# EBI-Metagenomics/deciphon-old

Measured on AMD Instinct MI355X. Metric: Gcell-updates/sec, higher is better.
Workload: dtype f32

## Files before the change

### deciphon-old_amd/__init__.py

```python
import ctypes as C
import os
import subprocess

import numpy as np

_HERE = os.path.dirname(os.path.abspath(__file__))
ROOT = os.path.dirname(_HERE)
LIB_PATH = os.path.join(_HERE, "libdcp_hip.so")
CSRC = os.path.join(_HERE, "csrc")

RC_OK, RC_END, RC_EFAIL, RC_EINVAL, RC_EIO, RC_ENOMEM, RC_EPARSE, RC_EAPI, RC_EHTTP = range(9)
RC_NAMES = ["RC_OK", "RC_END", "RC_EFAIL", "RC_EINVAL", "RC_EIO", "RC_ENOMEM", "RC_EPARSE",
            "RC_EAPI", "RC_EHTTP"]
ENTRY_DIST_NULL, ENTRY_DIST_UNIFORM, ENTRY_DIST_OCCUPANCY = 0, 1, 2
NCODES = 1364
NDIST = 129
NXTRANS = 13
CORE_SIZE_MAX = 4096
NUM_THREADS = 64

ABI_SYMBOLS = [
    "dcp_profile_new", "dcp_profile_sample", "dcp_profile_del", "dcp_profile_core_size",
    "dcp_profile_from_parts", "dcp_profile_entry_dist", "dcp_profile_epsilon", "dcp_rnd_seed", "dcp_rnd_next",
    "dcp_dist_unique_id", "dcp_dist_init", "dcp_dist_init_from_file", "dcp_dist_free", "dcp_dist_rank",
# ... 201 lines not shown
        "dcp_gpu_seqs_cut_windows": (I, [P, U, U]),
        "dcp_gpu_seqs_windows": (I, [P, C.POINTER(U), C.POINTER(U)]),
        "dcp_gpu_seqs_window_map": (I, [P, P, P, U]),
        "dcp_gpu_db_keep_dists": (I, [P, I]),
        "dcp_gpu_db_has_dists": (I, [P]),
        "dcp_gpu_decode_paths": (I, [P, P, P, U, P, P, P]),
        "dcp_profile_codon_joint": (I, [P, P, U, U, P, C.POINTER(C.c_double)]),
        "dcp_prod_format_row_codes": (C.c_long, [C.c_char_p, C.c_size_t, C.c_int64, C.c_int64, C.c_char_p, C.c_char_p,
                                                 C.c_double, C.c_double, C.c_char_p, C.c_char_p, P, P, U, P, U, P]),
        "dcp_gpu_path_domains": (I, [P, P, P, U, P, P, I, I, P, U, P, P, P, P]),
        "dcp_gpu_path_domains64": (I, [P, P, P, U, P, P, I, I, P, U, P, P, P, P]),
        "dcp_gpu_path_domains_kernel_ms": (F, [P]),
        "dcp_domains_locate": (I, [P, P, U, P, U, U, P, P, P, P, P, P]),
        "dcp_gpu_domains_locate": (I, [P, P, P, U, P, P, P, P]),
        "dcp_domains_merge": (I, [P, P, P, P, P, P, U, P, C.POINTER(U)]),
        "dcp_domains_regions": (I, [P, P, P, P, P, U, P, U, C.c_uint64, C.c_uint32, P, P, P, P, P, P, P, U, C.POINTER(U)]),
        "dcp_domains_locate_regions": (I, [P, P, U, P, U, P, P, P, P, P, P, P]),
        "dcp_gpu_seqs_cut_regions": (I, [P, P, P, P, P, U]),
        "dcp_gpu_seqs_regions": (U, [P]),
        "dcp_gpu_seqs_region_map": (I, [P, P, P, P, U]),
        "dcp_gpu_scan_pairs": (I, [P, C.POINTER(ScanParams), P, P, U]),
        "dcp_seq_random_thresholds": (I, [P, P]),
        "dcp_seq_random": (None, [C.c_uint64, C.c_uint32, U, P, P]),
        "dcp_gpu_seqs_random": (I, [P, U, U, C.c_uint64, P]),
        "dcp_gumbel_fit": (I, [P, U, C.c_size_t, C.POINTER(C.c_double), C.POINTER(C.c_double)]),
        "dcp_gpu_fit_gumbel": (I, [P, P, P, P]),
        "dcp_gpu_db_calibrate": (I, [P, U, U, C.c_uint64, P, I, I, I, P, P, P]),
        "dcp_gpu_calib_kernel_ms": (F, [P, I]),
        "dcp_gumbel_fit_tail": (I, [P, U, C.c_size_t, U, C.POINTER(C.c_double), C.POINTER(C.c_double),
                                    C.POINTER(C.c_double), C.POINTER(C.c_uint)]),
        "dcp_gpu_fit_gumbel_tail": (I, [P, U, P, P, P, P, P]),
        "dcp_gpu_db_calibrate_tail": (I, [P, U, U, C.c_uint64, P, I, I, I, U, P, P, P, P, P]),
        "dcp_gpu_calib_tail_kernel_ms": (F, [P, I]),
        "dcp_gumbel_sf": (C.c_double, [C.c_double, C.c_double, C.c_double]),
        "dcp_hits_evalues": (I, [P, U, P, P, P, U, C.c_double, P]),
        "dcp_hits_evalues64": (I, [P, U, P, P, P, U, C.c_double, P]),
        "dcp_forward_tables": (I, [U, U, P, P, P, P, P, P, U, C.POINTER(C.c_double), C.POINTER(C.c_double)]),
        "dcp_gpu_forward_pairs": (I, [P, I, I, P, P, U, P, P]),
        "dcp_gpu_forward_kernel_ms": (F, [P]),
        "dcp_posterior_tables": (I, [U, U, P, P, P, P, P, P, U, P, P, P, C.POINTER(C.c_double), C.POINTER(C.c_double)]),
        "dcp_posterior_envelopes": (I, [P, U, C.c_double, U, P, P, U, C.POINTER(U)]),
        "dcp_gpu_posterior_pairs": (I, [P, I, I, P, P, U, P, P, P, P, C.c_uint64, P, P]),
        "dcp_gpu_posterior_kernel_ms": (F, [P]),
        "dcp_mea_tables": (I, [U, U, P, P, P, P, P, P, U, P, U, C.POINTER(U), P, C.POINTER(C.c_double), C.POINTER(C.c_double)]),
        "dcp_mea_path_gain": (I, [U, U, P, P, P, P, P, P, U, P, U, C.POINTER(C.c_double), P]),
        "dcp_gpu_mea_pairs": (I, [P, I, I, P, P, U, P, U, P, P, P, P]),
        "dcp_gpu_mea_kernel_ms": (F, [P]),
        "dcp_gpu_forward_dense": (I, [P, I, I]),
        "dcp_fwd_factor_f32": (C.c_double, [C.c_float]),
        "dcp_forward_scaled_tables": (I, [U, U, P, P, P, P, P, P, U, I, C.POINTER(C.c_double), C.POINTER(C.c_double),
                                          C.POINTER(I)]),
        "dcp_forward_scaled_tables_band": (I, [U, U, P, P, P, P, P, P, U, I, I, C.POINTER(C.c_double), C.POINTER(C.c_double),
                                               C.POINTER(I)]),
        "dcp_gpu_forward_pairs_scaled": (I, [P, I, I, P, P, U, P, P]),
        "dcp_gpu_forward_scaled_redo_pairs": (U, [P]),
        "dcp_gpu_forward_scaled_kernel_ms": (F, [P]),
        "dcp_gpu_forward_dense_scaled": (I, [P, I, I]),
        "dcp_gpu_forward_dense_is_scaled": (I, [P]),
        "dcp_gpu_fetch_forward_scores": (I, [P, P, P]),
        "dcp_gpu_forward_dense_kernel_ms": (F, [P]),
        "dcp_exp_tail_fit": (I, [P, U, C.c_size_t, U, C.POINTER(C.c_double), C.POINTER(C.c_double),
                                 C.POINTER(C.c_double), C.POINTER(C.c_uint)]),
        "dcp_gpu_fit_exp_tail": (I, [P, I, U, P, P, P, P, P]),
        "dcp_gpu_exp_tail_kernel_ms": (F, [P, I]),
        "dcp_gpu_db_calibrate_forward": (I, [P, U, U, C.c_uint64, P, I, I, U, P, P, P, P, P]),
        "dcp_exp_sf": (C.c_double, [C.c_double, C.c_double, C.c_double]),
        "dcp_scores_evalues": (I, [P, P, P, U, P, P, P, U, C.c_double, I, P]),
    }
    if hooks:
        sig["dcp_gpu_test_set_redo_cap"] = (I, [P, U])
        sig["dcp_gpu_test_set_rowsweep_variant"] = (I, [P, I, U])
        sig["dcp_gpu_test_set_ring_stall"] = (I, [P, I])
        sig["dcp_gpu_test_set_seg_col_bytes"] = (I, [P, C.c_ulonglong])
        sig["dcp_gpu_test_set_trace_mode"] = (I, [P, I, C.c_ulonglong])
        sig["dcp_gpu_test_fetch_table_span"] = (I, [P, U, P, C.c_ulonglong, C.POINTER(U), C.POINTER(U), C.POINTER(U)])
        sig["dcp_gpu_test_fetch_seq_words"] = (I, [P, U, P, U, C.POINTER(U)])
        sig["dcp_gpu_test_last_rowsweep_plan"] = (I, [P, P, U, C.POINTER(U)])
        sig["dcp_gpu_test_last_pair_launches"] = (I, [P, P, U, C.POINTER(U)])
        sig["dcp_gpu_test_set_forward_waves"] = (I, [P, U])
        sig["dcp_gpu_test_set_dense_round"] = (I, [P, U])
        sig["dcp_gpu_test_set_forward_scale_band"] = (I, [P, U])
        sig["dcp_gpu_test_set_posterior_budget"] = (I, [P, C.c_ulonglong])
        sig["dcp_gpu_test_set_mea_budget"] = (I, [P, C.c_ulonglong])
    for name, (res, args) in sig.items():
        fn = getattr(lib, name)
        fn.restype = res
        fn.argtypes = args
    return lib


lib = _load()
TESTHOOKS_LIB_PATH = os.path.join(os.path.dirname(LIB_PATH), "libdcp_hip_testhooks.so")


def load_testhooks():
    return _load(TESTHOOKS_LIB_PATH, hooks=True)


def _f32(a):
    return np.ascontiguousarray(a, dtype=np.float32)


def _f64(a):
    return np.ascontiguousarray(a, dtype=np.float64)


class ProteinCfg:

    def __init__(self, entry_dist=ENTRY_DIST_OCCUPANCY, epsilon=0.01):
        if not (0.0 <= epsilon <= 1.0):
            raise DcpError(RC_EINVAL, "epsilon out of [0, 1]")
        self.entry_dist = entry_dist
        self.epsilon = float(np.float32(epsilon))
        self.epsilon64 = float(epsilon)


PROTEIN_CFG_DEFAULT = ProteinCfg(ENTRY_DIST_OCCUPANCY, 0.01)


class ProteinProfile:

    def __init__(self, handle):
        if not handle:
            raise DcpError(RC_EINVAL, "profile construction failed")
        self._h = handle

    def __del__(self):
        h, self._h = getattr(self, "_h", None), None
        if h:
            lib.dcp_profile_del(h)

    @classmethod
    def sample(cls, seed, core_size, cfg=PROTEIN_CFG_DEFAULT, accession="accession", precision=32):
        rc = C.c_int(0)
        if precision == 64:
            h = lib.dcp_profile_sample64(accession.encode(), seed, core_size, cfg.entry_dist,
                                         cfg.epsilon64, C.byref(rc))
        elif precision == 32:
            h = lib.dcp_profile_sample(accession.encode(), seed, core_size, cfg.entry_dist,
                                       cfg.epsilon, C.byref(rc))
        else:
            raise DcpError(RC_EINVAL, "precision is 32 or 64")
        if not h:
            raise DcpError(rc.value, "protein_profile_sample")
        return cls(h)

    @classmethod
    def from_params(cls, null_lprobs, match_lprobs, trans, cfg=PROTEIN_CFG_DEFAULT,
                    accession="accession", consensus=None, precision=32):
        if precision not in (32, 64):
            raise DcpError(RC_EINVAL, "precision is 32 or 64")
        cv = _f64 if precision == 64 else _f32
        nl, ml, tr = cv(null_lprobs), cv(match_lprobs), cv(trans)
        M = ml.shape[0] if ml.ndim == 2 else 0
        if nl.shape != (20,) or ml.shape != (M, 20) or tr.shape != (M + 1, 7):
            raise DcpError(RC_EINVAL, "bad parameter shapes")
        rc = C.c_int(0)
        cons = consensus.encode() if consensus else None
        new, eps = (lib.dcp_profile_new64, cfg.epsilon64) if precision == 64 else (lib.dcp_profile_new, cfg.epsilon)
        h = new(accession.encode(), M, cfg.entry_dist, eps, nl.ctypes.data, ml.ctypes.data, tr.ctypes.data, cons,
                C.byref(rc))
        if not h:
            raise DcpError(rc.value, "protein_model_setup")
        return cls(h)

    @property
# ... 922 lines not shown
                                                           lam.ctypes.data, status.ctypes.data, tau.ctypes.data,
                                                           k_eff.ctypes.data))
        self._seq_lens = np.full(n, length, np.int64)
        return mu, lam, status, tau, k_eff

    def test_set_dense_round(self, npairs):
        self._check(self._lib.dcp_gpu_test_set_dense_round(self._c, int(npairs)))

    def posterior_pairs(self, seq_idx, profile_idx, multi_hits=True, hmmer3_compat=False):
        sq, pr = _pair_list(seq_idx, profile_idx)
        lens = getattr(self, "_seq_lens", np.zeros(0, np.int64))
        ok = sq < len(lens)
        cap = int(np.sum(lens[sq[ok]] + 1)) if len(sq) else 0
        row_off = np.zeros(len(sq) + 1, np.uint64)
        begin, end, core = (np.zeros(cap, np.float64) for _ in range(3))
        fwd, bwd = np.zeros(len(sq), np.float64), np.zeros(len(sq), np.float64)
        self._check(self._lib.dcp_gpu_posterior_pairs(self._c, int(multi_hits), int(hmmer3_compat), sq.ctypes.data,
                                                      pr.ctypes.data, len(sq), row_off.ctypes.data, begin.ctypes.data,
                                                      end.ctypes.data, core.ctypes.data, cap, fwd.ctypes.data,
                                                      bwd.ctypes.data))
        return row_off, begin, end, core, fwd, bwd

    @property
    def posterior_kernel_ms(self):
        return self._lib.dcp_gpu_posterior_kernel_ms(self._c)

    def test_set_posterior_budget(self, nbytes):
        self._check(self._lib.dcp_gpu_test_set_posterior_budget(self._c, int(nbytes)))

    def mea_pairs(self, seq_idx, profile_idx, multi_hits=True, hmmer3_compat=False):
        sq, pr = _pair_list(seq_idx, profile_idx)
        n = len(sq)
        lens = self._seq_lens
        sizes = np.array([p.core_size for p in self._profiles or []], np.int64)
        ok = (sq < len(lens)) & (pr < len(sizes))
        cap = int(np.sum(lens[sq[ok]] + sizes[pr[ok]] + 16))
        off = np.zeros(n + 1, np.uint32)
        gain, fwd = np.zeros(n, np.float64), np.zeros(n, np.float64)
        for _ in range(2):
            steps, post = np.zeros(max(cap, 1), STEP_DTYPE), np.zeros(max(cap, 1), np.float64)
            rc = self._lib.dcp_gpu_mea_pairs(self._c, int(multi_hits), int(hmmer3_compat), sq.ctypes.data, pr.ctypes.data, n,
                                             steps.ctypes.data, cap, off.ctypes.data, post.ctypes.data, gain.ctypes.data,
                                             fwd.ctypes.data)
            if rc != RC_ENOMEM or int(off[n]) <= cap:
                break
            cap = int(off[n])
        self._check(rc)
        paths = [steps[int(off[i]):int(off[i + 1])].copy() for i in range(n)]
        posts = [post[int(off[i]):int(off[i + 1])].copy() for i in range(n)]
        return paths, posts, gain, fwd

    @property
    def mea_kernel_ms(self):
        return self._lib.dcp_gpu_mea_kernel_ms(self._c)

    def test_set_mea_budget(self, nbytes):
        self._check(self._lib.dcp_gpu_test_set_mea_budget(self._c, int(nbytes)))

    def set_hit_buffer(self, hits_dev_ptr, cap, nhits_dev_ptr):
        self._check(self._lib.dcp_gpu_set_hit_buffer(self._c, hits_dev_ptr, cap, nhits_dev_ptr))

    def set_hit_buffer64(self, hits_dev_ptr, cap, nhits_dev_ptr):
        self._check(self._lib.dcp_gpu_set_hit_buffer64(self._c, hits_dev_ptr, cap, nhits_dev_ptr))

    def hit_buffer64(self):
        h, n, cap = C.c_void_p(), C.c_void_p(), C.c_uint(0)
        self._check(self._lib.dcp_gpu_hit_buffer64(self._c, C.byref(h), C.byref(n), C.byref(cap)))
        return h.value, n.value, cap.value

    def launch_infos(self):
        out = []
        for i in range(self.last_scan_launches):
            li = LaunchInfo()
            self._check(self._lib.dcp_gpu_last_scan_launch_info(self._c, i, C.byref(li)))
            out.append(dict(R=li.nodes_per_lane, W=li.waves_per_pair, nprofiles=li.nprofiles,
                            ms=li.ms, cells=li.cells, algorithmic_bytes=li.algorithmic_bytes))
        return out

    def sync(self):
        self._check(self._lib.dcp_gpu_sync(self._c))

    def test_set_redo_cap(self, cap):
        self._check(self._lib.dcp_gpu_test_set_redo_cap(self._c, int(cap)))

    def test_set_ring_stall(self, on):
        self._check(self._lib.dcp_gpu_test_set_ring_stall(self._c, int(bool(on))))

    def test_set_seg_col_bytes(self, nbytes):
        self._check(self._lib.dcp_gpu_test_set_seg_col_bytes(self._c, int(nbytes)))

    def test_set_trace_mode(self, own_forward, budget_floats=0):
        self._check(self._lib.dcp_gpu_test_set_trace_mode(self._c, int(bool(own_forward)), int(budget_floats)))

    def test_table_span(self, p):
        span, ldk, eb = C.c_uint(0), C.c_uint(0), C.c_uint(0)
        self._check(self._lib.dcp_gpu_test_fetch_table_span(self._c, p, None, 0, C.byref(span), C.byref(ldk),
                                                            C.byref(eb)))
        out = np.zeros((NCODES, span.value), np.float64 if eb.value == 8 else np.float32)
        self._check(self._lib.dcp_gpu_test_fetch_table_span(self._c, p, out.ctypes.data, out.nbytes, C.byref(span),
                                                            C.byref(ldk), C.byref(eb)))
        return out, ldk.value

    def test_rowsweep_plan(self):
        n = C.c_uint(0)
        rc = self._lib.dcp_gpu_test_last_rowsweep_plan(self._c, None, 0, C.byref(n))
        if rc != RC_ENOMEM:
            self._check(rc or RC_EFAIL)
        w = np.zeros(n.value, np.uint32)
        self._check(self._lib.dcp_gpu_test_last_rowsweep_plan(self._c, w.ctypes.data, len(w), C.byref(n)))
        per = (len(w) - 2) // int(w[1])
        classes = {}
        for k in range(int(w[1])):
            R, W, path, stage, waves, pf, chunk, redo, rest = (int(v) for v in w[2 + per * k:2 + per * k + 9])
            if path:
                classes[(R, W)] = dict(path=("plain", "mp", "segmented")[path - 1], stage=stage, waves=waves, prefetch=pf,
                                       chunk=chunk, seg_redo=redo, flagged_rest=bool(rest))
        return dict(forked=bool(w[0]), classes=classes)

    def test_pair_launches(self):
        n = C.c_uint(0)
        rc = self._lib.dcp_gpu_test_last_pair_launches(self._c, None, 0, C.byref(n))
        if rc != RC_ENOMEM:
            self._check(rc or RC_EFAIL)
        w = np.zeros(n.value, np.uint32)
        self._check(self._lib.dcp_gpu_test_last_pair_launches(self._c, w.ctypes.data, len(w), C.byref(n)))
        out = []
        for i in range(int(w[0])):
            kind, prec, a, b, units, tpb, cap = (int(v) for v in w[1 + 7 * i:8 + 7 * i])
            rec = dict(kind=("scan_pairs", "qlane_redo", "seg_redo")[kind - 1], precision=prec, units=units, tpb=tpb, cap=cap)
            rec.update(dict(cls=(a, b)) if prec == 32 else dict(group=a, R=b))
            out.append(rec)
        return out

    def test_set_rowsweep_variant(self, stage_rows, block_waves=0):
        self._check(self._lib.dcp_gpu_test_set_rowsweep_variant(self._c, int(stage_rows), int(block_waves)))

    @property
    def last_scan_ms(self):
        return self._lib.dcp_gpu_last_scan_ms(self._c)

    @property
    def last_scan_kernel(self):
        return self._lib.dcp_gpu_last_scan_kernel(self._c)

    @property
    def last_scan_launches(self):
        return self._lib.dcp_gpu_last_scan_launches(self._c)

    @property
    def last_scan_query_plan(self):
        nb, rows, prow, mg = C.c_uint(0), C.c_ulonglong(0), C.c_uint(0), C.c_uint(0)
        self._check(self._lib.dcp_gpu_last_scan_query_plan(self._c, C.byref(nb), C.byref(rows), C.byref(prow),
                                                           C.byref(mg)))
        return dict(nblocks=nb.value, sum_block_rows=rows.value, plane_rows=prow.value,
                    max_groups_per_slot=mg.value)

    @property
    def last_scan_redo_pairs(self):
        n = C.c_uint(0)
        self._check(self._lib.dcp_gpu_last_scan_redo_pairs(self._c, C.byref(n)))
        return n.value

    @property
    def cells(self):
        return self._lib.dcp_gpu_scan_cells(self._c)

# ... 110 lines not shown
```

### deciphon-old_amd/csrc/dcp_gpu.hip

```cpp
#include "dcp_kernels.h"
#include "dcp_f64.h"
#include "dcp_seqs.h"
#include "dcp_decode.h"
#include "dcp_domains.h"
#include "dcp_calib.h"
#include "dcp_forward.h"
#include "dcp_forward_scaled.h"
#include "dcp_mea.h"
#include "dcp_posterior.h"
#include "dcp_test_hooks.h"

#include <hip/hip_runtime.h>

#include <algorithm>
#include <cmath>
#include <cstdarg>
#include <cstdio>
#include <cstring>
#include <limits>
#include <map>
#include <new>
#include <numeric>
#include <string>
#include <queue>
// ... 48 lines not shown
    }
    hipError_t reserve(size_t count) { return n < count ? alloc(count) : hipSuccess; }
    void release()
    {
        if (p) (void)hipFree(p);
        p = nullptr;
        n = 0;
    }
    ~DevBuf() { release(); }
};

template <class Real, class Hit> struct ScanResults
{
    DevBuf<Real> d_null, d_alt;
    DevBuf<Hit> d_hits;
    DevBuf<unsigned> d_nhits;
    unsigned hit_cap = 0;
    bool have_scores = false;
    Hit *ext_hits = nullptr;
    unsigned *ext_nhits = nullptr;
    unsigned ext_cap = 0;
    Hit *hits() const { return ext_hits ? ext_hits : d_hits.p; }
    unsigned *nhits() const { return ext_hits ? ext_nhits : d_nhits.p; }
    unsigned cap() const { return ext_hits ? ext_cap : hit_cap; }
    hipError_t ensure(size_t npairs, bool keep_scores)
    {
        hipError_t e = hipSuccess;
        if (keep_scores && d_null.n != npairs)
        {
            if ((e = d_null.alloc(npairs)) != hipSuccess) return e;
            if ((e = d_alt.alloc(npairs)) != hipSuccess) return e;
        }
        have_scores = keep_scores;
        unsigned const want_cap = (unsigned)std::min<size_t>(npairs, (size_t)1 << 22);
        if (!ext_hits && hit_cap < want_cap)
        {
            if ((e = d_hits.alloc(want_cap)) != hipSuccess) return e;
            hit_cap = want_cap;
        }
        return d_nhits.p ? hipSuccess : d_nhits.alloc(1);
    }
    void release()
    {
        d_null.release(), d_alt.release(), d_hits.release(), d_nhits.release();
        hit_cap = 0;
        have_scores = false;
    }
};

bool is_nan(float v)
{
    uint32_t bits;
    std::memcpy(&bits, &v, sizeof bits);
    return (bits & 0x7fffffffu) > 0x7f800000u;
}
bool is_nan(double v)
{
    uint64_t bits;
    std::memcpy(&bits, &v, sizeof bits);
    return (bits & 0x7fffffffffffffffull) > 0x7ff0000000000000ull;
}

constexpr int kMaxLaunches = 2 * kNumClasses + 1;

struct LastScan
{
    bool scanned = false;
    bool f64 = false;
    bool pair_scan = false;
    unsigned q0 = 0, q1 = 0;
    int kernel = 0;
    int kernel_variant = 0;
    struct dcp_scan_params prm = {};
    unsigned launches = 0;
    unsigned n_launched = 0;
    int launched_class[kMaxLaunches] = {0};
    bool launched_redo[kMaxLaunches] = {false};
    bool overlapped = false;
    unsigned redo_pairs = 0;
    uint64_t pair_cells = 0, pair_bytes = 0;
    uint64_t pair_class_cells[DCP_MAX_CLASSES] = {0}, pair_class_bytes[DCP_MAX_CLASSES] = {0};
    bool redo_pending = false, redo_pending64 = false, ring_check_pending = false;
#ifdef DCP_TEST_HOOKS
    struct RowsweepClassPlan
    {
        unsigned path = 0;
        unsigned stage = 0, waves = 0, prefetch = 0;
        unsigned chunk = 0;
        unsigned flagged_rest = 0;
    } rs_plan[kNumClasses];
    struct PairLaunch
    {
        unsigned kind, precision, a, b, units, tpb, cap;
    };
    std::vector<PairLaunch> pair_launches;
#endif
};

}

struct dcp_gpu_ctx
{
    int device = 0;
    hipStream_t stream = nullptr;
    hipEvent_t ev_start = nullptr, ev_stop = nullptr;
    std::string err;

    unsigned nprof = 0;
    std::vector<dcp_prof_meta> metas;
    std::vector<unsigned> core_sizes;
    unsigned class_first[kNumClasses + 1] = {0};
    DevBuf<dcp_prof_meta> d_metas;
    DevBuf<uint32_t> d_slot_of_pidx;
    std::vector<uint32_t> slot_of_pidx;
    DevBuf<float> d_emis_match, d_emis_insert, d_emis_null, d_trans8;
    DevBuf<float> d_dists, d_eps;
    std::vector<dcp_expand_tile> rs_tiles;
    uint64_t rs_floats = 0;
    bool rs_ready = false;
    bool one_layout = false;
    uint64_t table_bytes = 0;
    int ql_G = 2;
    std::vector<dcp_ql_prof> ql_metas;
    uint64_t sum_core = 0, sum_tiles = 0;
    uint64_t class_core[DCP_MAX_CLASSES] = {0};
    unsigned max_tiles = 0;
    DevBuf<dcp_ql_prof> d_ql_metas;
    DevBuf<float> d_emis_tiles, d_ttrans, d_scratch;
    DevBuf<uint32_t> d_qorder;
    DevBuf<uint32_t> d_words_t, d_wt_off;
    std::vector<dcp_mp_group> mp_groups;
    unsigned mp_first[3] = {0, 0, 0};
    unsigned mp_flagged_first[2] = {0, 0};
    DevBuf<dcp_mp_group> d_mp_groups;
    DevBuf<float> d_mp_in;
    bool mp_in_ready = false;
    DevBuf<dcp_ql_group> d_ql_groups;
    DevBuf<uint32_t> d_slot_first;
    unsigned ql_nqb = 0, ql_plane_rows = 0;
    unsigned ring_stall = 0;
    uint32_t *h_qstage = nullptr;
    size_t h_qstage_n = 0;
    hipEvent_t ev_qstage = nullptr;
    int rs_force_stg = -1;
    unsigned rs_force_bw = 0;
    unsigned rs_pad_lds = 0;
    int rs_force_pf = 0;
    int rs_force_R = 0;
    bool any_exact_e = false;
    DevBuf<unsigned> d_task_counter;
    DevBuf<dcp_pair> d_redo;
    DevBuf<unsigned> d_redo_n;
    unsigned qorder_q0 = ~0u, qorder_q1 = ~0u, qorder_lmax = 0;
    unsigned num_cus = 0;
    unsigned qorder_nt = 0;
    unsigned redo_cap_limit = 1u << 26;
    float last_ql_ms = 0;

    unsigned nseqs = 0;
    unsigned strands = 0;
    uint64_t total_len = 0;
    std::vector<uint32_t> seq_len;
    unsigned win_window = 0, win_step = 0;
    std::vector<uint32_t> win_src, win_off;
    std::vector<uint32_t> reg_src, reg_begin;
    std::vector<uint8_t> reg_minus;
    void drop_windows()
    {
        win_window = win_step = 0;
        win_src.clear(), win_off.clear();
        reg_src.clear(), reg_begin.clear(), reg_minus.clear();
    }
    DevBuf<uint32_t> d_seq_words, d_seq_woff, d_seq_len;
    DevBuf<float> d_xtrans;
    int xt_multi = -1, xt_h3 = -1;
    bool xt_explicit = false;
    std::vector<double> xt64;

    ScanResults<float, dcp_hit> res;
    LastScan last;
    DevBuf<dcp_pair> d_pair_list;
    DevBuf<unsigned> d_pair_n;
    hipEvent_t ev_class[kMaxLaunches] = {nullptr};
    hipStream_t class_stream[kNumClasses] = {nullptr};
    hipEvent_t ev_trace[kNumClasses + 1] = {nullptr};
    DevBuf<float> d_trace_work;
    int trace_mode = 0;
    uint64_t trace_budget = 0;
    DevBuf<float> d_seg_scratch;
    DevBuf<dcp_pair> d_seg_redo;
    DevBuf<unsigned> d_seg_redo_n;
    int seg_mode = -1;
    int mp_mode = -1;
    uint64_t seg_col_bytes = (uint64_t)6 << 30;

    int precision = 0;
    double lrt_threshold64 = std::numeric_limits<double>::quiet_NaN();
    struct F64Db
    {
        std::vector<dcp_f64_prof> profs;
        std::vector<uint32_t> slot_of_pidx;
        unsigned group_first[5] = {0, 0, 0, 0, 0};
        DevBuf<dcp_f64_prof> d_profs;
        DevBuf<double> d_tab, d_trans, d_xe;
        DevBuf<double> d_xt, d_col;
        ScanResults<double, dcp_hit64> res;
        DevBuf<uint32_t> d_order, d_qorder, d_slot_first;
        DevBuf<dcp_ql_group> d_groups;
        unsigned plan_blocks = 0, plan_rows = 0, plan_max_groups = 0;
        uint64_t plan_sum_rows = 0;
        DevBuf<double> d_planes;
        DevBuf<unsigned> d_task, d_redo_n;
        DevBuf<dcp_f64_pair> d_redo;
        DevBuf<dcp_f64_pair> d_pair_list;
        DevBuf<unsigned> d_pair_n;
        void release()
        {
            d_pair_list.release(), d_pair_n.release();
            profs.clear();
            d_profs.release(), d_tab.release(), d_trans.release(), d_xe.release();
            d_xt.release(), d_col.release(), res.release();
            d_order.release(), d_qorder.release(), d_planes.release(), d_task.release(), d_redo_n.release();
            d_redo.release(), d_slot_first.release(), d_groups.release();
            slot_of_pidx.clear();
        }
    } f64;

    bool keep_dists = false;
    struct DecodeDb
    {
        bool ready = false;
        DevBuf<double> d_dists64;
        DevBuf<uint32_t> d_match_row;
        DevBuf<double> d_exp, d_eps;
        void release()
// ... 2277 lines not shown
    HIP_TRY(c, hipMemcpyAsync(c->d_qorder.p, h_ord, nq * sizeof(uint32_t), hipMemcpyHostToDevice, c->stream));
    HIP_TRY(c, hipMemcpyAsync(c->d_wt_off.p, wt_off, (nqb + 1u) * sizeof(uint32_t), hipMemcpyHostToDevice, c->stream));
    HIP_TRY(c, hipMemcpyAsync(c->d_slot_first.p, h_slots, nslot_words * sizeof(uint32_t), hipMemcpyHostToDevice, c->stream));
    HIP_TRY(c, hipMemcpyAsync(c->d_ql_groups.p, h_groups, ngroup_words * sizeof(uint32_t), hipMemcpyHostToDevice, c->stream));
    HIP_TRY(c, hipEventRecord(c->ev_qstage, c->stream));
    dcp_qlane_args ta{};
    ta.seq_words = a.seq_words, ta.seq_woff = a.seq_woff, ta.seq_len = a.seq_len;
    ta.qorder = c->d_qorder.p, ta.words_t = c->d_words_t.p, ta.wt_off = c->d_wt_off.p;
    ta.groups = c->d_ql_groups.p, ta.slot_first = c->d_slot_first.p;
    ta.nseqs = nq, ta.nqblocks = nqb;
    if (dcp_launch_qlane_transpose(&ta, NTq, c->stream)) return c->fail(DCP_EFAIL, "no kernel for %u-query blocks", NTq);
    HIP_TRY(c, hipGetLastError());
    c->qorder_q0 = q_begin, c->qorder_q1 = q_end, c->qorder_nt = NTq;
    c->ql_nqb = nqb, c->ql_plane_rows = plan.plane_rows + 8u;
    return DCP_OK;
}

static int record_launch(dcp_gpu_ctx *c, int k, bool is_redo, hipStream_t stream, bool join)
{
    HIP_TRY(c, hipEventRecord(c->ev_class[c->last.n_launched], stream));
    if (join) HIP_TRY(c, hipStreamWaitEvent(c->stream, c->ev_class[c->last.n_launched], 0));
    c->last.launched_redo[c->last.n_launched] = is_redo;
    c->last.launched_class[c->last.n_launched++] = k;
    c->last.launches++;
    return DCP_OK;
}

static int launch_qlane_scan(dcp_gpu_ctx *c, struct dcp_scan_params const *prm, dcp_scan_args &a, unsigned NT,
                             unsigned ql_blocks_per_cu, bool two_stage, bool use_w3)
{
    dcp_qlane_args qa{};
    qa.profs = c->d_ql_metas.p;
    qa.emis_tiles = c->one_layout ? c->d_emis_match.p : c->d_emis_tiles.p;
    qa.tiles_from_rows = c->one_layout ? 1u : 0u;
    qa.emis_insert = c->d_emis_insert.p;
    qa.emis_null = c->d_emis_null.p;
    qa.ttrans = c->d_ttrans.p;
    qa.seq_words = a.seq_words;
    qa.seq_woff = a.seq_woff;
    qa.seq_len = a.seq_len;
    qa.xtrans = a.xtrans;
    qa.qorder = c->d_qorder.p;
    qa.words_t = c->d_words_t.p;
    qa.wt_off = c->d_wt_off.p;
    qa.groups = c->d_ql_groups.p;
    qa.slot_first = c->d_slot_first.p;
    qa.ring_stall = c->ring_stall;
    qa.task_counter = c->d_task_counter.p;
    qa.out_null = a.out_null;
    qa.out_alt = a.out_alt;
    qa.hits = a.hits;
    qa.nhits = a.nhits;
    qa.hit_cap = a.hit_cap;
    qa.lrt_threshold = prm->lrt_threshold;
    qa.nprof = c->nprof;
    qa.nprof_total = c->nprof;
    qa.nseqs = a.nseqs;
    qa.q_base = a.q_base;
    qa.plane_rows = c->ql_plane_rows;
    qa.nqblocks = c->ql_nqb;
    uint64_t const ntasks = (uint64_t)c->nprof * qa.nqblocks;
    if (ntasks > 0xffffffffull) return c->fail(DCP_EINVAL, "scan too large for one launch");
    qa.ntasks = (unsigned)ntasks;
    bool const redo = prm->multi_hits != 0 || c->xt_explicit || (dcp_qlane_exact_e_by_redo() && c->any_exact_e);
    unsigned redo_grid[kNumClasses] = {0};
    if (redo)
    {
        if (int rc = ensure_rowsweep_layout(c)) return rc;
        a.emis_match = c->d_emis_match.p;
        uint64_t tot = 0;
        uint64_t const cap_limit = c->redo_cap_limit;
        for (int k = 0; k < kNumClasses; ++k)
        {
            uint64_t const pairs = (uint64_t)a.nseqs * (c->class_first[k + 1] - c->class_first[k]);
            unsigned const cap = (unsigned)std::min<uint64_t>(pairs, cap_limit);
            qa.redo_base[k] = (unsigned)tot;
            qa.redo_cap[k] = cap;
            tot += cap;
            uint64_t const tpb = dcp_rowsweep_tasks_per_block(kClasses[k].W);
            uint64_t g = std::min<uint64_t>((cap + tpb - 1) / tpb, 8ull * c->num_cus);
            redo_grid[k] = (unsigned)((g + 7) / 8 * 8);
        }
        HIP_TRY(c, c->d_redo.reserve((size_t)tot));
    }
    HIP_TRY(c, c->d_redo_n.reserve(DCP_MAX_CLASSES + 2));
    HIP_TRY(c, hipMemsetAsync(c->d_redo_n.p, 0, (DCP_MAX_CLASSES + 2) * sizeof(unsigned), c->stream));
    qa.redo = c->d_redo.p;
    qa.redo_n = c->d_redo_n.p;
    qa.redo_overflow = c->d_redo_n.p + DCP_MAX_CLASSES;
    qa.ring_error = c->d_redo_n.p + DCP_MAX_CLASSES + 1;
    uint64_t const per_block = (uint64_t)dcp_qlane_scratch_planes() * (uint64_t)qa.plane_rows * NT;
    uint64_t const budget = (uint64_t)64 << 28;
    uint64_t fit = per_block ? budget / per_block : 0;
    uint64_t const resident_blocks = (uint64_t)ql_blocks_per_cu * c->num_cus;
    unsigned nblocks = (unsigned)std::min<uint64_t>(std::min<uint64_t>(ntasks, resident_blocks), fit);
    if (use_w3) nblocks = (nblocks + 2u) / 3u * 3u;
    if (nblocks == 0)
        return c->fail(DCP_ENOMEM, "sequences too long for the query-lane kernel (%u plane rows): use kernel = 1", qa.plane_rows);
    size_t const need = (size_t)nblocks * per_block;
    HIP_TRY(c, c->d_scratch.reserve(need));
    qa.scratch = c->d_scratch.p;
    HIP_TRY(c, hipMemsetAsync(c->d_task_counter.p, 0, sizeof(unsigned), c->stream));
    HIP_TRY(c, hipEventRecord(c->ev_start, c->stream));
    if (two_stage ? dcp_launch_qlane2(&qa, nblocks, c->stream)
                  : use_w3 ? dcp_launch_qlane_w3(&qa, nblocks / 3u, c->stream)
                           : dcp_launch_qlane(&qa, nblocks, NT, c->stream))
        return c->fail(DCP_EFAIL, "query-lane launch failed");
    HIP_TRY(c, hipGetLastError());
    if (int rc = record_launch(c, -1, false, c->stream, false)) return rc;
    for (int k = 0; redo && k < kNumClasses; ++k)
    {
        if (redo_grid[k] == 0) continue;
        a.pairs = c->d_redo.p + qa.redo_base[k];
        a.npairs = c->d_redo_n.p + k;
        a.pair_cap = qa.redo_cap[k];
        a.first_prof = 0;
        a.nprof = c->nprof;
        SizeClass const sc = kClasses[k];
        if (dcp_launch_rowsweep(sc.R, sc.W, &a, redo_grid[k], c->stream))
            return c->fail(DCP_EFAIL, "no kernel for class R=%d W=%d", sc.R, sc.W);
        if (int rc = record_launch(c, k, true, c->stream, false)) return rc;
        note_pair_launch(c, DCP_PL_QLANE_REDO, 32u, (unsigned)sc.R, (unsigned)sc.W, redo_grid[k], dcp_rowsweep_tasks_per_block(sc.W), a.pair_cap);
    }
    HIP_TRY(c, hipGetLastError());
    HIP_TRY(c, hipEventRecord(c->ev_stop, c->stream));
    c->last.redo_pending = redo;
    c->last.ring_check_pending = two_stage;
    c->last.scanned = true;
    return DCP_OK;
}

struct SegSweepPlan
{
    unsigned stride = 0;
    unsigned chunk[kNumClasses] = {0};
    uint64_t redo_off[kNumClasses] = {0}, col_rows = 0, redo_tot = 0;
};
static SegSweepPlan plan_segsweep(dcp_gpu_ctx const *c, unsigned q_begin, unsigned q_end)
{
    SegSweepPlan sp;
    unsigned const nq = q_end - q_begin;
    sp.stride = *std::max_element(c->seq_len.begin() + q_begin, c->seq_len.begin() + q_end) + 2u;
    for (int k = 0; k < kNumClasses; ++k)
    {
        unsigned const np = c->class_first[k + 1] - c->class_first[k];
        SizeClass const sc = kClasses[k];
        uint64_t const pairs = (uint64_t)np * nq;
        bool const want = c->seg_mode == 1 || (c->seg_mode < 0 && pairs >= 16ull * c->num_cus);
        bool const have = sc.W > 1 && want && np > 0 && pairs <= ((uint64_t)1 << 26);
        if (!have) continue;
        uint64_t const per_query = (uint64_t)np * 2u * sp.stride * 16u;
        uint64_t const chunk = std::min<uint64_t>(nq, c->seg_col_bytes / per_query);
        if (chunk == 0) continue;
        if ((uint64_t)np * ((chunk + 3u) / 4u) > 0x7ffffff0ull) continue;
        sp.chunk[k] = (unsigned)chunk;
        sp.col_rows += (uint64_t)np * chunk * 2u * sp.stride;
        sp.redo_off[k] = sp.redo_tot, sp.redo_tot += pairs;
    }
    return sp;
}

static int launch_segsweep_class(dcp_gpu_ctx *c, dcp_scan_args &a, int k, SegSweepPlan const &sp, float *col_base,
                                 hipStream_t ls, bool overlap)
{
    unsigned const first = a.first_prof, last = first + a.nprof, np = a.nprof, chunk = sp.chunk[k], nq = a.nseqs;
    uint64_t const ntasks = (uint64_t)a.nprof * a.nchunks;
    SizeClass const sc = kClasses[k];
    a.seg_stride = sp.stride;
    a.seg_redo = c->d_seg_redo.p + sp.redo_off[k];
    a.seg_redo_n = c->d_seg_redo_n.p + k;
    a.seg_redo_cap = (unsigned)ntasks;
    for (unsigned sub = first; sub < last;)
    {
        unsigned const segR = seg_r_of(c->metas[sub].core_size);
        unsigned sub_end = sub, max_m = 0;
        while (sub_end < last && seg_r_of(c->metas[sub_end].core_size) == segR)
            max_m = std::max(max_m, c->metas[sub_end].core_size), ++sub_end;
        unsigned const nsub = sub_end - sub, nseg_max = (max_m + 64u * segR - 1u) / (64u * segR);
        a.first_prof = sub, a.nprof = nsub;
        a.seg_col0 = col_base + (size_t)(sub - first) * chunk * 2u * sp.stride * 4u;
        a.seg_col1 = a.seg_col0 + (size_t)nsub * chunk * sp.stride * 4u;
        for (unsigned qc = 0; qc < nq; qc += chunk)
        {
            a.seg_q0 = qc, a.seg_nq = std::min(chunk, nq - qc);
            for (unsigned sg = 0; sg < nseg_max; ++sg)
            {
                a.seg_index = sg;
                if (dcp_launch_segsweep((int)segR, &a, dcp_segsweep_blocks(nsub, a.seg_nq), ls))
                    return c->fail(DCP_EFAIL, "no segmented kernel for %u nodes per lane", segR);
            }
        }
        sub = sub_end;
    }
    a.first_prof = first, a.nprof = np;
    if (int rc = record_launch(c, k, false, ls, false)) return rc;
    a.pairs = a.seg_redo, a.npairs = a.seg_redo_n, a.pair_cap = a.seg_redo_cap;
    a.first_prof = 0, a.nprof = c->nprof;
    uint64_t g = std::min<uint64_t>(ntasks, 8ull * c->num_cus);
    g = (g + 7u) / 8u * 8u;
    if (dcp_launch_rowsweep(sc.R, sc.W, &a, (unsigned)g, ls))
        return c->fail(DCP_EFAIL, "no kernel for class R=%d W=%d", sc.R, sc.W);
    note_pair_launch(c, DCP_PL_SEG_REDO, 32u, (unsigned)sc.R, (unsigned)sc.W, (unsigned)g, dcp_rowsweep_tasks_per_block(sc.W), a.pair_cap);
    return record_launch(c, k, true, ls, overlap);
}

static int launch_rowsweep_scan(dcp_gpu_ctx *c, dcp_scan_args &a, unsigned q_begin, unsigned q_end)
{
    unsigned const nq = q_end - q_begin;
// ... 979 lines not shown
    if (segmented) HIP_TRY(c, hipMemcpy(redo, c->d_seg_redo_n.p, sizeof redo, hipMemcpyDeviceToHost));
    out[0] = c->last.overlapped ? 1u : 0u;
    out[1] = (unsigned)kNumClasses;
    for (int k = 0; k < kNumClasses; ++k)
    {
        unsigned *w = out + 2u + DCP_RS_PLAN_WORDS * (unsigned)k;
        LastScan::RowsweepClassPlan const &r = c->last.rs_plan[k];
        w[0] = (unsigned)kClasses[k].R, w[1] = (unsigned)kClasses[k].W, w[2] = r.path, w[3] = r.stage, w[4] = r.waves;
        w[5] = r.prefetch, w[6] = r.chunk, w[7] = r.path == DCP_RS_PATH_SEGMENTED ? redo[k] : 0u, w[8] = r.flagged_rest;
    }
    return DCP_OK;
}
int dcp_gpu_test_last_pair_launches(dcp_gpu_ctx *c, unsigned *out, unsigned cap, unsigned *nwords)
{
    if (!c || !nwords) return DCP_EINVAL;
    if (!c->last.scanned) return c->fail(DCP_EINVAL, "no scan yet");
    *nwords = 1u + DCP_PL_WORDS * (unsigned)c->last.pair_launches.size();
    if (!out || cap < *nwords) return DCP_ENOMEM;
    HIP_TRY(c, hipSetDevice(c->device));
    HIP_TRY(c, hipStreamSynchronize(c->stream));
    out[0] = (unsigned)c->last.pair_launches.size();
    unsigned *w = out + 1u;
    for (LastScan::PairLaunch const &l : c->last.pair_launches)
    {
        w[0] = l.kind, w[1] = l.precision, w[2] = l.a, w[3] = l.b, w[4] = l.units, w[5] = l.tpb, w[6] = l.cap;
        w += DCP_PL_WORDS;
    }
    return DCP_OK;
}
int dcp_gpu_test_set_seg_col_bytes(dcp_gpu_ctx *c, unsigned long long bytes)
{
    if (!c) return DCP_EINVAL;
    c->seg_col_bytes = bytes ? bytes : (uint64_t)6 << 30;
    return DCP_OK;
}
int dcp_gpu_test_set_ring_stall(dcp_gpu_ctx *c, int on)
{
    if (!c) return DCP_EINVAL;
    c->ring_stall = on ? 1u : 0u;
    return DCP_OK;
}
int dcp_gpu_test_set_trace_mode(dcp_gpu_ctx *c, int own_forward, unsigned long long budget_floats)
{
    if (!c) return DCP_EINVAL;
    c->trace_mode = own_forward ? 1 : 0;
    c->trace_budget = budget_floats;
    return DCP_OK;
}
int dcp_gpu_test_set_posterior_budget(dcp_gpu_ctx *c, unsigned long long bytes)
{
    if (!c) return DCP_EINVAL;
    c->sweeps.post_budget = bytes;
    return DCP_OK;
}

int dcp_gpu_test_set_mea_budget(dcp_gpu_ctx *c, unsigned long long bytes)
{
    if (!c) return DCP_EINVAL;
    c->sweeps.mea_budget = bytes;
    return DCP_OK;
}

int dcp_gpu_test_set_forward_waves(dcp_gpu_ctx *c, unsigned nwaves)
{
    if (!c) return DCP_EINVAL;
    c->sweeps.waves_cap = nwaves;
    return DCP_OK;
}

int dcp_gpu_test_set_forward_scale_band(dcp_gpu_ctx *c, unsigned bits)
{
    if (!c || bits > 500u) return DCP_EINVAL;
    c->sweeps.band = (int)bits;
    return DCP_OK;
}

int dcp_gpu_test_set_dense_round(dcp_gpu_ctx *c, unsigned npairs)
{
    if (!c) return DCP_EINVAL;
    c->sweeps.dense_round = npairs;
    return DCP_OK;
}

int dcp_gpu_test_set_redo_cap(dcp_gpu_ctx *c, unsigned cap)
{
    if (!c) return DCP_EINVAL;
    c->redo_cap_limit = cap ? cap : 1u << 26;
    return DCP_OK;
}
int dcp_gpu_test_fetch_table_span(dcp_gpu_ctx *c, unsigned p, void *out, unsigned long long cap_bytes,
                                  unsigned *span, unsigned *ldk, unsigned *elem_bytes)
{
    if (!c || !span || !ldk || !elem_bytes || p >= c->nprof) return DCP_EINVAL;
    HIP_TRY(c, hipSetDevice(c->device));
    void const *src = nullptr;
    unsigned w = 0, ld = 0, eb = 0;
    if (c->precision == 64)
    {
        for (dcp_f64_prof const &m : c->f64.profs)
            if (m.pidx == p) src = c->f64.d_tab.p + m.tab_off, w = m.ldk, ld = m.ldk, eb = sizeof(double);
    }
    else
    {
        if (int rc = ensure_rowsweep_layout(c)) return rc;
        for (dcp_prof_meta const &m : c->metas)
            if (m.pidx == p) src = c->d_emis_match.p + m.emis_off, w = m.width, ld = m.ldk, eb = sizeof(float);
    }
    if (!src) return DCP_EINVAL;
    *span = w, *ldk = ld, *elem_bytes = eb;
    if (!out) return DCP_OK;
    if (cap_bytes < (unsigned long long)DCP_NCODES * w * eb) return c->fail(DCP_ENOMEM, "span needs more room");
    HIP_TRY(c, hipMemcpy2D(out, (size_t)w * eb, src, (size_t)ld * eb, (size_t)w * eb, DCP_NCODES, hipMemcpyDeviceToHost));
    return DCP_OK;
}
#endif

int dcp_gpu_sync(dcp_gpu_ctx *c)
{
    if (!c) return DCP_EINVAL;
    HIP_TRY(c, hipSetDevice(c->device));
    return finish_scan(c);
}

int dcp_gpu_last_scan_redo_pairs(dcp_gpu_ctx *c, unsigned *npairs)
{
    if (!c || !npairs) return DCP_EINVAL;
    if (!c->last.scanned) return c->fail(DCP_EINVAL, "no scan yet");
    HIP_TRY(c, hipSetDevice(c->device));
    if (int rc = finish_scan(c)) return rc;
    *npairs = c->last.redo_pairs;
    return DCP_OK;
}

int dcp_gpu_last_scan_query_plan(dcp_gpu_ctx *c, unsigned *nblocks, unsigned long long *sum_block_rows,
                                 unsigned *plane_rows, unsigned *max_groups_per_slot)
{
    if (!c) return DCP_EINVAL;
    if (!c->last.scanned) return c->fail(DCP_EINVAL, "no scan yet");
    HIP_TRY(c, hipSetDevice(c->device));
    if (int rc = finish_scan(c)) return rc;
    if (!c->last.f64 || c->last.kernel_variant != 4)
        return c->fail(DCP_EINVAL, "the last scan did not run the f64 query-lane kernel (kernel = 4): it has no batch plan");
    if (nblocks) *nblocks = c->f64.plan_blocks;
    if (sum_block_rows) *sum_block_rows = c->f64.plan_sum_rows;
    if (plane_rows) *plane_rows = c->f64.plan_rows;
    if (max_groups_per_slot) *max_groups_per_slot = c->f64.plan_max_groups;
    return DCP_OK;
}

float dcp_gpu_last_scan_ms(dcp_gpu_ctx *c)
{
    if (!c || !c->last.scanned) return -1.0f;
    float ms = -1.0f;
    if (hipEventSynchronize(c->ev_stop) != hipSuccess) return -1.0f;
    if (hipEventElapsedTime(&ms, c->ev_start, c->ev_stop) != hipSuccess) return -1.0f;
    return ms;
}

unsigned dcp_gpu_last_scan_launches(dcp_gpu_ctx const *c) { return c ? c->last.launches : 0; }
int dcp_gpu_last_scan_kernel(dcp_gpu_ctx const *c) { return c && c->last.scanned ? c->last.kernel_variant : 0; }

int dcp_gpu_last_scan_launch_info(dcp_gpu_ctx *c, unsigned i, struct dcp_launch_info *out)
{
    if (!c || !out || !c->last.scanned) return DCP_EINVAL;
    if (i >= c->last.n_launched) return DCP_EINVAL;
    int const k = c->last.launched_class[i];
// ... 742 lines not shown
```

### deciphon-old_amd/csrc/dcp_kernels.h

```cpp
#ifndef DCP_KERNELS_H
#define DCP_KERNELS_H

#include "dcp_host.h"
#include <stdint.h>

struct dcp_prof_meta
{
    uint64_t emis_off;
    uint32_t trans_off;
    uint32_t core_size;
    uint32_t ldk;
    uint32_t pidx;
    uint32_t flags;
    uint32_t width;
};
#define DCP_PROF_EXACT_E 1u

struct dcp_mp_group
{
    uint64_t emis_off;
    uint32_t trans_off;
    uint32_t ldk;
    uint32_t in_off;
    uint32_t nparts;
    uint32_t col0[4];
    uint32_t core_size[4];
    uint32_t pidx[4];
    uint32_t slot[4];
};

struct dcp_pair
{
    uint32_t q;
    uint32_t slot;
};
#define DCP_MAX_CLASSES 16

struct dcp_scan_args
{
    dcp_prof_meta const *profs;
    float const *emis_match;
    float const *emis_insert;
    float const *emis_null;
    float const *trans8;
    uint32_t const *seq_words;
    uint32_t const *seq_woff;
    uint32_t const *seq_len;
    float const *xtrans;
    float *out_null;
    float *out_alt;
    dcp_hit *hits;
    unsigned *nhits;
    unsigned hit_cap;
    float lrt_threshold;
    unsigned first_prof;
    unsigned nprof;
    unsigned nprof_total;
    unsigned nseqs;
    unsigned q_base;
    unsigned qchunk;
    unsigned nchunks;
    dcp_pair const *pairs;
    unsigned const *npairs;
    unsigned pair_cap;
    float *seg_col0, *seg_col1;
    unsigned seg_stride;
    unsigned seg_index;
    dcp_mp_group const *mp_groups;
    float const *mp_in;
    unsigned seg_q0, seg_nq;
    dcp_pair *seg_redo;
    unsigned *seg_redo_n;
    unsigned seg_redo_cap;
    float *trace_work;
    uint64_t const *trace_woff;
    float *trace_alt;
};

struct dcp_expand_tile
{
    uint64_t out_off;
    uint32_t dist_row;
    uint32_t ncols;
    uint32_t nstore;
    uint32_t ld_code;
    uint32_t ld_col;
    uint32_t kt;
    uint32_t col0;
};

enum : uint32_t
{
    DCP_TRACE_NO_PATH = 0xffffffffu,
    DCP_TRACE_TOO_LONG = 0xfffffffeu,
};
struct dcp_trace_args
{
    dcp_prof_meta const *profs;
    uint32_t const *slot_of_pidx;
    float const *emis_match;
    float const *emis_insert;
    float const *emis_null;
    float const *trans8;
    uint32_t const *seq_words;
    uint32_t const *seq_woff;
    uint32_t const *seq_len;
    float const *xtrans;
    dcp_hit const *hits;
    unsigned nhits;
    float *work;
    uint64_t const *work_off;
    dcp_step *steps;
    uint32_t const *step_off;
    uint32_t *nsteps;
    float *alt_out;
    int null_model;
    int skip_forward;
    uint32_t const *work_ld;
};

struct dcp_ql_prof
{
    uint64_t tile_off;
    uint32_t ttrans_off;
    uint32_t core_size;
    uint32_t ntiles;
    uint32_t pidx;
    uint32_t rs_slot;
    uint32_t cls;
    uint32_t needs_exact_e;
    uint32_t ldk;
};

struct dcp_ql_group
{
    uint32_t qfirst;
    uint32_t nq;
    uint32_t rowbase;
    uint32_t lmax;
};

struct dcp_qlane_args
{
    dcp_ql_prof const *profs;
    float const *emis_tiles;
    float const *emis_insert;
    float const *emis_null;
    float const *ttrans;
    uint32_t const *seq_words;
    uint32_t const *seq_woff;
    uint32_t const *seq_len;
    float const *xtrans;
    uint32_t const *qorder;
    dcp_ql_group const *groups;
    uint32_t const *slot_first;
    uint32_t *words_t;
    uint32_t const *wt_off;
    float *scratch;
    unsigned *task_counter;
    unsigned *ring_error;
    unsigned ring_stall;
    dcp_pair *redo;
    unsigned *redo_n;
    unsigned *redo_overflow;
    unsigned redo_base[DCP_MAX_CLASSES];
    unsigned redo_cap[DCP_MAX_CLASSES];
    float *out_null;
    float *out_alt;
    dcp_hit *hits;
    unsigned *nhits;
    unsigned hit_cap;
    float lrt_threshold;
    unsigned nprof;
    unsigned nprof_total;
    unsigned nseqs;
    unsigned q_base;
    unsigned plane_rows;
    unsigned ntasks;
    unsigned nqblocks;
    unsigned tiles_from_rows;
};

struct dcp_expand_args
{
    dcp_expand_tile const *tiles;
    float const *dists;
    float const *eps;
    float *out;
};

#ifdef __cplusplus
extern "C" {
#endif
void dcp_launch_expand(dcp_expand_args const *a, unsigned ntiles, void *stream);
int dcp_launch_rowsweep(int R, int W, dcp_scan_args const *a, unsigned nblocks,
                        void *stream);
unsigned dcp_rowsweep_tasks_per_block(int W);
int dcp_launch_segsweep(int R, dcp_scan_args const *a, unsigned nblocks, void *stream);
int dcp_launch_mp(int K, dcp_scan_args const *a, void *stream);
void dcp_launch_mp_in(dcp_mp_group const *groups, unsigned ngroups, unsigned n_first, unsigned k_first, unsigned k_rest,
                      float const *emis_insert, float const *emis_null, float *out, void *stream);
unsigned dcp_segsweep_blocks(unsigned nprof, unsigned nq);
int dcp_launch_rowsweep_grid(int R, int W, dcp_scan_args const *a, int stg, unsigned bw, void *stream,
                             unsigned pad_lds,
                             int prefetch2);
unsigned dcp_rowsweep_max_block_waves(int R, int W, int stg);
unsigned dcp_rowsweep_stage_bytes(int R, int stg);
int dcp_launch_qlane(dcp_qlane_args const *a, unsigned nblocks, unsigned nt, void *stream);
int dcp_launch_qlane2(dcp_qlane_args const *a, unsigned nblocks, void *stream);
unsigned dcp_qlane2_lds_bytes(void);
int dcp_launch_qlane_w3(dcp_qlane_args const *a, unsigned nblocks, void *stream);
int dcp_launch_qlane_transpose(dcp_qlane_args const *a, unsigned nt, void *stream);
void dcp_launch_trace(dcp_trace_args const *a, unsigned nhits, void *stream);
int dcp_launch_trace_forward(int R, int W, dcp_scan_args const *a, unsigned nblocks, void *stream);
unsigned dcp_qlane_block_size(void);
unsigned dcp_qlane_tile_nodes(void);
unsigned dcp_qlane_scratch_planes(void);
unsigned dcp_qlane_diag_build(void);
unsigned dcp_qlane_group_rows(unsigned lmax);
unsigned dcp_qlane_window_planes(void);
unsigned dcp_qlane_exact_e_by_redo(void);
#ifdef __cplusplus
}
#endif

#ifdef __HIP__
__device__ inline __attribute__((always_inline)) bool dcp_lrt_hit(float nul, float alt, float thr)
{
    auto finite = [](float v) { return (__builtin_bit_cast(unsigned, v) & 0x7f800000u) != 0x7f800000u; };
    float const lrt = -2 * (nul - alt);
    return finite(nul) && finite(alt) && finite(lrt) && !(lrt < thr);
}
#endif

#endif
```

### deciphon-old_amd/csrc/dcp_kernels.hip

```cpp
#include "dcp_kernels.h"

#include <hip/hip_runtime.h>
#include <algorithm>

namespace
{

__device__ __forceinline__ float neg_inf() { return -__builtin_inff(); }

typedef float const __attribute__((address_space(4))) cfloat;
typedef uint32_t const __attribute__((address_space(4))) cu32;
__device__ __forceinline__ cfloat *as_const(float const *p) { return (cfloat *)(unsigned long long)p; }
__device__ __forceinline__ cu32 *as_const(uint32_t const *p) { return (cu32 *)(unsigned long long)p; }

template <int CTRL, int ROW_MASK, int BANK_MASK>
__device__ __forceinline__ float dpp_mov(float old_value, float v)
{
    return __builtin_bit_cast(
        float, __builtin_amdgcn_update_dpp(__builtin_bit_cast(int, old_value),
                                           __builtin_bit_cast(int, v), CTRL,
                                           ROW_MASK, BANK_MASK, false));
}

__device__ __forceinline__ float lane_shr1(float v, float first)
// ... 138 lines not shown
};
template <> struct VecLoad<6>
{
    static __device__ __forceinline__ void ld(float const *p, float (&o)[6])
    {
        float t[3], u[3];
        VecLoad<3>::ld(p, t);
        VecLoad<3>::ld(p + 3, u);
        o[0] = t[0], o[1] = t[1], o[2] = t[2], o[3] = u[0], o[4] = u[1], o[5] = u[2];
    }
};
template <> struct VecLoad<7>
{
    static __device__ __forceinline__ void ld(float const *p, float (&o)[7])
    {
        struct __attribute__((packed, aligned(4))) f4 { float x, y, z, w; };
        f4 v = *reinterpret_cast<f4 const *>(p);
        float u[3];
        VecLoad<3>::ld(p + 4, u);
        o[0] = v.x, o[1] = v.y, o[2] = v.z, o[3] = v.w, o[4] = u[0], o[5] = u[1], o[6] = u[2];
    }
};
template <> struct VecLoad<8>
{
    static __device__ __forceinline__ void ld(float const *p, float (&o)[8])
    {
        float4 v = *reinterpret_cast<float4 const *>(p);
        float4 w = *reinterpret_cast<float4 const *>(p + 4);
        o[0] = v.x, o[1] = v.y, o[2] = v.z, o[3] = v.w, o[4] = w.x, o[5] = w.y, o[6] = w.z, o[7] = w.w;
    }
};

__device__ __forceinline__ unsigned code_of(unsigned w, int l)
{
    constexpr unsigned off[5] = {0u, 4u, 20u, 84u, 340u};
    return off[l - 1] + (w & ((1u << (2 * l)) - 1u));
}

template <int R> struct PairState
{
    float P[5][R];
    float Q[5][R];
    float PX[5];
};

struct LaneSpecial
{
    float a;
    float b;
    float c;
};

template <int R> struct Trans
{
    float ent[R], mm[R], im[R], dm[R], md[R], dd[R], mi[R], ii[R];
};

struct RowOut
{
    float E;
    float X;
};

template <int W> struct Exchange
{
    float m[2][W], i[2][W], d[2][W], e[2][W];
    int flag[3];
};

template <int R, int r = 1>
__device__ __forceinline__ void chain_rest(float const (&a)[R], float (&d)[R], float const (&dd)[R])
{
    if constexpr (r < R)
    {
        d[r] = fmaxf(a[r], d[r - 1] + dd[r]);
        chain_rest<R, r + 1>(a, d, dd);
    }
}

struct NoSink
{
    template <class... A> __device__ __forceinline__ void operator()(A const &...) const {}
};
template <int R, int W, int PH, int PARTS = 1, class Fetch, class Sink = NoSink>
__device__ __forceinline__ RowOut dp_row(PairState<R> &s, Trans<R> const &t,
                                         float (&em)[5][R], float (&em3)[R], float (&em4)[R], float (&em5)[R], float (&eN)[5], float (&eI)[5],
                                         LaneSpecial const &sp, float const xEB,
                                         Exchange<(W > 1 ? W : 1)> *xc,
                                         unsigned wave, unsigned lane,
                                         unsigned &gen, unsigned const exact_e, Fetch &&fetch, Sink &&sink = Sink{})
{
    constexpr int s1 = (PH + 4) % 5, s2 = (PH + 3) % 5, s3 = (PH + 2) % 5,
                  s4 = (PH + 1) % 5, s5 = PH;
    float const ni = neg_inf();

    float m[R], ins[R];
#pragma unroll
    for (int r = 0; r < R; ++r)
    {
        m[r] = max5(s.P[s1][r] + em[0][r], s.P[s2][r] + em[1][r],
                    s.P[s3][r] + em3[r], s.P[s4][r] + em4[r],
                    s.P[s5][r] + em5[r]);
        ins[r] = max5(s.Q[s1][r] + eI[0], s.Q[s2][r] + eI[1], s.Q[s3][r] + eI[2],
                      s.Q[s4][r] + eI[3], s.Q[s5][r] + eI[4]);
    }
    float const X = max5(s.PX[s1] + eN[0], s.PX[s2] + eN[1], s.PX[s3] + eN[2],
                         s.PX[s4] + eN[3], s.PX[s5] + eN[4]);
    __builtin_amdgcn_sched_barrier(0);
    fetch();
    __builtin_amdgcn_sched_barrier(0);

    float E = ni;
    if constexpr (W == 1)
    {
        float em = m[0];
#pragma unroll
        for (int r = 1; r < R; ++r)
            em = fmaxf(em, m[r]);
        if constexpr (PARTS == 1) E = wave_max(em);
        else E = part_max<PARTS>(em);
    }

    float m_first = ni, i_first = ni, d_first = ni;
    constexpr bool XW = W > 1;
    float a[R], d[R];
#pragma unroll
    for (int r = 1; r < R; ++r)
        a[r] = m[r - 1] + t.md[r];
    auto refine = [&]() {
        if constexpr (W == 1)
        {
            for (;;)
            {
                float const c0 = shr1_add<XW>(d[R - 1], d_first, t.dd[0]);
                unsigned long long changed;
                asm("v_cmp_gt_f32_e64 %0, %2, %1\n\t"
                    "v_max_f32_e32 %1, %1, %2"
                    : "=&s"(changed), "+v"(d[0])
                    : "v"(c0));
                if (changed == 0ull) break;
                chain_rest<R>(a, d, t.dd);
            }
        }
        else
        {
            a[0] = shr1_add<XW>(m[R - 1], m_first, t.md[0]);
            for (;;)
            {
                float const d0 = fmaxf(a[0], shr1_add<XW>(d[R - 1], d_first, t.dd[0]));
                if (!__any(d0 != d[0])) break;
                d[0] = d0;
                chain_rest<R>(a, d, t.dd);
            }
        }
    };
    auto lane_max = [&]() {
        float e = fmaxf(m[0], d[0]);
#pragma unroll
        for (int r = 1; r < R; ++r)
            e = fmaxf(e, fmaxf(m[r], d[r]));
        return e;
    };
    d[0] = shr1_add<XW>(m[R - 1], m_first, t.md[0]);
    chain_rest<R>(a, d, t.dd);
    refine();

    if constexpr (W == 1)
    {
        unsigned xe = exact_e;
        asm volatile("" : "+s"(xe));
        if (__builtin_expect(xe != 0u, 0))
        {
            float ed = d[0];
#pragma unroll
            for (int r = 1; r < R; ++r)
                ed = fmaxf(ed, d[r]);
            E = __builtin_bit_cast(float, __builtin_amdgcn_readfirstlane(__builtin_bit_cast(int, fmaxf(E, wave_max(ed)))));
        }
    }
    else
    {
        float published = ni;
        float e_m = m[0];
#pragma unroll
        for (int r = 1; r < R; ++r)
            e_m = fmaxf(e_m, m[r]);
        e_m = wave_max(e_m);
        for (unsigned it = 0;; ++it, ++gen)
        {
            unsigned const buf = gen & 1u;
            float const e_wave = exact_e ? wave_max(lane_max()) : e_m;
            if (lane == 63)
            {
                if (it == 0)
                {
                    xc->m[buf][wave] = m[R - 1];
                    xc->i[buf][wave] = ins[R - 1];
                }
                else if (d[R - 1] != published)
                    xc->flag[gen % 3u] = 1;
                xc->d[buf][wave] = d[R - 1];
// ... 122 lines not shown
__device__ __forceinline__ unsigned base_at(uint32_t const *__restrict__ words, unsigned pos)
{
    return (words[pos >> 4] >> ((pos & 15u) * 2u)) & 3u;
}

typedef char const __attribute__((address_space(1))) *gchar_ptr;
typedef float const __attribute__((address_space(3))) *lds_cfloat_ptr;
template <int R, int STAGED, int LMASK = 31, bool SCALARS = true>
__device__ __forceinline__ void load_row(float const *__restrict__ em_base,
                                         unsigned ldk, unsigned &lane_boff,
                                         cfloat *eN_tab, cfloat *eI_tab,
                                         unsigned w, float (&em)[5][R], float (&em3)[R], float (&em4)[R], float (&em5)[R],
                                         float (&eN)[5], float (&eI)[5], float const *stg, unsigned stg_ldk = 0u)
{
    unsigned const sldk = stg_ldk ? stg_ldk : ldk;
    asm volatile("" : "+v"(lane_boff));
#pragma unroll
    for (int l = 1; l <= 5; ++l)
    {
        unsigned const c = code_of(w, l);
        if ((LMASK >> (l - 1)) & 1)
        {
            float(&dst)[R] = l == 3 ? em3 : l == 4 ? em4 : l == 5 ? em5 : em[l - 1];
            if (STAGED > 0 && (l == 1 ? 4 : l == 2 ? 20 : l == 3 ? 84 : 1364) <= STAGED)
            {
                unsigned roff = c * sldk * 4u;
                asm volatile("" : "+s"(roff));
                VecLoad<R>::ld((float const *)((char const *)stg + (roff + lane_boff)), dst);
            }
            else
            {
                gchar_ptr row = (gchar_ptr)em_base + c * ldk * 4u;
                asm volatile("" : "+s"(row));
                VecLoad<R>::ld((float const *)(row + lane_boff), dst);
            }
        }
        if (SCALARS)
        {
            eN[l - 1] = eN_tab[c];
            eI[l - 1] = eI_tab[c];
        }
    }
}

}

#ifndef DCP_RS_R4_WAVES
#define DCP_RS_R4_WAVES 4
#endif
#ifndef DCP_RS_R2_WAVES
#define DCP_RS_R2_WAVES 6
#endif
#ifndef DCP_RS_R5_WAVES
#define DCP_RS_R5_WAVES 3
#endif
#ifndef DCP_RS_R6_WAVES
#define DCP_RS_R6_WAVES 3
#endif
#ifndef DCP_RS_R7_WAVES
#define DCP_RS_R7_WAVES 2
#endif
#ifndef DCP_RS_R4_BIG_WAVES
#define DCP_RS_R4_BIG_WAVES DCP_RS_R4_WAVES
#endif
#ifndef DCP_RS_PAIR_BIG
#define DCP_RS_PAIR_BIG 0
#endif
#ifndef DCP_RS_R2_BIG_WAVES
#define DCP_RS_R2_BIG_WAVES 7
#endif
#ifndef DCP_RS_R3_BIG_WAVES
#define DCP_RS_R3_BIG_WAVES 5
#endif
constexpr int rs_min_waves(int R, int W = 1, bool big = false)
{
    return R == 2 ? (big ? DCP_RS_R2_BIG_WAVES : DCP_RS_R2_WAVES) : R == 3 && W == 1 && big ? DCP_RS_R3_BIG_WAVES : R <= 3 ? 4
           : R == 4 ? (W == 1 ? (big ? DCP_RS_R4_BIG_WAVES : DCP_RS_R4_WAVES) : 4)
           : R == 5 ? (big ? DCP_RS_R5_WAVES : 2) : R == 6 ? (big ? DCP_RS_R6_WAVES : 2) : R == 7 ? DCP_RS_R7_WAVES : 2;
}
constexpr int rs_block_threads(int R, int W, int STG, bool PF = false)
{
    return W > 1 ? 64 * W : STG > 0 ? (rs_min_waves(R, W, STG == 20 && !PF) >= 4 ? 1024 : 256 * rs_min_waves(R, W, STG == 20 && !PF)) : 256;
}
template <int R, int W, int STG, bool PF, bool TRACE = false>
__global__ __launch_bounds__(rs_block_threads(R, W, STG, PF), TRACE ? (W > 4 ? 1 : 2) : rs_min_waves(R, W, (STG == 20 && !PF) || (STG == 0 && W == 1 && DCP_RS_PAIR_BIG))) void viterbi_rowsweep_kernel(dcp_scan_args a)
{
    static_assert(!PF || STG > 0, "only staged variants prefetch two rows ahead");
    static_assert(!TRACE || (STG == 0 && !PF), "the traceback's forward pass is an unstaged pair-mode kernel");
    static_assert(W == 1 || STG == 0, "only one-wavefront pairs stage rows");
    constexpr unsigned TASKS_PER_BLOCK = (W == 1 && STG == 0) ? 4u : 1u;
    constexpr int STAGED = STG;
    constexpr bool PF2 = PF;
    constexpr int NEAR = STG >= 84 ? 7 : 3, FAR = 31 - NEAR;
    __shared__ Exchange<(W > 1 ? W : 1)> xc_mem;
    __shared__ __attribute__((aligned(16))) float stage_mem[STAGED > 0 ? STAGED * (64 * R + (R <= 2 ? 8 : 0)) : 4];
    float const *const stg = stage_mem;
    Exchange<(W > 1 ? W : 1)> *xc = &xc_mem;
    unsigned const lane = threadIdx.x & 63u;
    unsigned const wave = __builtin_amdgcn_readfirstlane(threadIdx.x >> 6);

    unsigned const nblk = gridDim.x;
    unsigned const vblk = (blockIdx.x & 7u) * (nblk >> 3) + (blockIdx.x >> 3);
    bool const pair_mode = STAGED > 0 ? false : a.pairs != nullptr;
    unsigned const bw = STAGED > 0 ? blockDim.x >> 6 : 1u;
    unsigned const bpp = STAGED > 0 ? (a.nchunks + bw - 1u) / bw : 1u;
    unsigned task = TASKS_PER_BLOCK > 1u ? vblk * TASKS_PER_BLOCK + wave : vblk;
    unsigned const ntasks = pair_mode ? min(*a.npairs, a.pair_cap) : STAGED > 0 ? a.nprof * bpp : a.nprof * a.nchunks;
    for (; task < ntasks; task += nblk * TASKS_PER_BLOCK)
    {
    unsigned slot, q0, q1;
    if (pair_mode)
    {
        dcp_pair const pr = a.pairs[task];
        slot = pr.slot, q0 = pr.q, q1 = pr.q + 1u;
    }
    else if constexpr (STAGED > 0)
    {
        unsigned const s_rel = task / bpp;
        unsigned const chunk = (task - s_rel * bpp) * bw + wave;
        slot = a.first_prof + s_rel;
        q0 = min(chunk * a.qchunk, a.nseqs);
        q1 = min(q0 + a.qchunk, a.nseqs);
    }
    else
    {
        unsigned const s_rel = task / a.nchunks;
        slot = a.first_prof + s_rel;
        q0 = (task - s_rel * a.nchunks) * a.qchunk;
        q1 = min(q0 + a.qchunk, a.nseqs);
    }
    slot = __builtin_amdgcn_readfirstlane(slot);
    q0 = __builtin_amdgcn_readfirstlane(q0);
    q1 = __builtin_amdgcn_readfirstlane(q1);

    dcp_prof_meta const pm = a.profs[slot];
    float const *__restrict__ em_base = a.emis_match + pm.emis_off;
    cfloat *eN_tab = as_const(a.emis_null + (size_t)pm.pidx * DCP_NCODES);
    cfloat *eI_tab = as_const(a.emis_insert + (size_t)pm.pidx * DCP_NCODES);
    unsigned const ldk = pm.ldk;
    unsigned const exact_e = __builtin_amdgcn_readfirstlane(pm.flags & DCP_PROF_EXACT_E);
    unsigned const node0 = (W == 1 ? lane : wave * 64u + lane) * R;
    unsigned const m4 = (pm.core_size + 3u) & ~3u;
    unsigned const lane_off = node0 < pm.core_size ? node0 : (m4 + R <= pm.width ? m4 : pm.width - R);
    unsigned gen = 0;
    unsigned const swd = pm.width;
    if constexpr (STAGED > 0)
    {
        unsigned const n4 = swd >> 2;
        for (unsigned i = threadIdx.x; i < (unsigned)STAGED * n4; i += blockDim.x)
        {
            unsigned const c = i / n4, k = i - c * n4;
            reinterpret_cast<float4 *>(stage_mem + c * swd)[k] = reinterpret_cast<float4 const *>(em_base + (size_t)c * ldk)[k];
        }
        __syncthreads();
    }
    if constexpr (W > 1)
    {
        __syncthreads();
        if (threadIdx.x == 0) xc->flag[0] = xc->flag[1] = xc->flag[2] = 0;
        __syncthreads();
    }

    Trans<R> t;
    {
        float const *__restrict__ tb = a.trans8 + pm.trans_off + lane_off;
        VecLoad<R>::ld(tb + (size_t)DCP_T_ENTRY * ldk, t.ent);
        VecLoad<R>::ld(tb + (size_t)DCP_T_MM * ldk, t.mm);
        VecLoad<R>::ld(tb + (size_t)DCP_T_IM * ldk, t.im);
        VecLoad<R>::ld(tb + (size_t)DCP_T_DM * ldk, t.dm);
        VecLoad<R>::ld(tb + (size_t)DCP_T_MD * ldk, t.md);
        VecLoad<R>::ld(tb + (size_t)DCP_T_DD * ldk, t.dd);
        VecLoad<R>::ld(tb + (size_t)DCP_T_MI * ldk, t.mi);
        VecLoad<R>::ld(tb + (size_t)DCP_T_II * ldk, t.ii);
    }

    for (unsigned q = q0; q < q1; ++q)
    {
        unsigned const L = a.seq_len[q];
        cu32 *words = as_const(a.seq_words + a.seq_woff[q]);
        cfloat *xt = as_const(a.xtrans + (size_t)q * DCP_XSTRIDE);
        float const ni = neg_inf();
        unsigned const x = lane & 3u;
        LaneSpecial sp;
        sp.a = x == 1u ? xt[DCP_X_EJ] : x == 2u ? xt[DCP_X_EC] : ni;
        sp.b = x == 0u ? xt[DCP_X_NN] : x == 1u ? xt[DCP_X_JJ] : x == 2u ? xt[DCP_X_CC] : xt[DCP_X_RR];
        sp.c = x == 0u ? xt[DCP_X_NB] : x == 1u ? xt[DCP_X_JB] : ni;
        float xEB = xt[DCP_X_EB];
        asm volatile("" : "+v"(xEB));

        PairState<R> s;
#pragma unroll
        for (int h = 0; h < 5; ++h)
        {
#pragma unroll
            for (int r = 0; r < R; ++r)
                s.P[h][r] = ni, s.Q[h][r] = ni;
            s.PX[h] = ni;
        }
        {
            float const B0 = 0.0f + xt[DCP_X_SB];
#pragma unroll
            for (int r = 0; r < R; ++r)
                s.P[0][r] = B0 + t.ent[r];
            s.PX[0] = x == 0u ? 0.0f + xt[DCP_X_SN] : x == 3u ? 0.0f : ni;
        }

        float em[5][R], eN[5], eI[5];
        RowOut o{ni, ni};
        unsigned j = 1;
        unsigned lane_boff = lane_off * 4u;
        constexpr unsigned RW = 64u * R * W;
        float *t_m = nullptr, *t_x = nullptr, *t_e = nullptr;
        size_t t_mat = 0;
        unsigned t_rows = 0;
        if constexpr (TRACE)
        {
            float *const work = a.trace_work + a.trace_woff[task];
            t_rows = L + 1u;
            t_mat = (size_t)t_rows * RW;
            t_m = work + node0;
            float *const spec = work + 3u * t_mat;
#pragma unroll
            for (int r = 0; r < R; ++r)
                t_m[r] = ni, t_m[t_mat + r] = ni, t_m[2u * t_mat + r] = ni;
            t_m += RW;
            t_x = spec + (x == 0u ? 0u : x == 1u ? 3u * t_rows : 4u * t_rows);
            t_e = spec;
            if ((W == 1 || wave == 0u) && lane < 3u) t_x[0] = ni;
            if ((W == 1 || wave == 0u) && lane == 0u) t_e[t_rows] = 0.0f + xt[DCP_X_SB], t_e[2u * t_rows] = ni;
            ++t_x, ++t_e;
        }
        auto const sink = [&](float const(&m_)[R], float const(&i_)[R], float const(&d_)[R], float E_, float X_, float B_) {
            if constexpr (TRACE)
            {
#pragma unroll
                for (int r = 0; r < R; ++r)
                    t_m[r] = m_[r], t_m[t_mat + r] = i_[r], t_m[2u * t_mat + r] = d_[r];
                t_m += RW;
                if ((W == 1 || wave == 0u) && lane < 3u) *t_x = X_;
                if ((W == 1 || wave == 0u) && lane == 0u) t_e[t_rows] = B_, t_e[2u * t_rows] = E_;
                ++t_x, ++t_e;
            }
        };
        if constexpr (PF2)
        {
            float emg[2][3][R];
            unsigned w1 = base_at(words, 0);
            unsigned w2 = ((w1 << 2) | base_at(words, 1)) & 1023u;
            load_row<R, STAGED, NEAR, true>(em_base, ldk, lane_boff, eN_tab, eI_tab, w1, em, em[2], em[3], em[4], eN, eI, stg, swd);
            load_row<R, STAGED, FAR, false>(em_base, ldk, lane_boff, eN_tab, eI_tab, w1, em, emg[1][0], emg[1][1], emg[1][2], eN, eI, stg, swd);
            load_row<R, STAGED, FAR, false>(em_base, ldk, lane_boff, eN_tab, eI_tab, w2, em, emg[0][0], emg[0][1], emg[0][2], eN, eI, stg, swd);
#define DCP_E3(PAR) (STG >= 84 ? em[2] : emg[PAR][0])
#define DCP_ROW2(PH, PAR)                                                      \
    {                                                                          \
        w1 = w2;                                                \
        w2 = ((w2 << 2) | base_at(words, j + 1u)) & 1023u;      \
        o = dp_row<R, W, PH>(s, t, em, DCP_E3(PAR), emg[PAR][1], emg[PAR][2], eN, eI, sp, xEB, xc, wave, lane, gen, exact_e, [&]() { \
            load_row<R, STAGED, NEAR, true>(em_base, ldk, lane_boff, eN_tab, eI_tab, w1, em, em[2], em[3], em[4], eN, eI, stg, swd); \
            load_row<R, STAGED, FAR, false>(em_base, ldk, lane_boff, eN_tab, eI_tab, w2, em, emg[PAR][0], emg[PAR][1], emg[PAR][2], eN, eI, stg, swd); \
        });                                                                    \
        ++j;                                                                   \
    }
            while (j + 9 <= L)
            {
                DCP_ROW2(1, 1) DCP_ROW2(2, 0) DCP_ROW2(3, 1) DCP_ROW2(4, 0) DCP_ROW2(0, 1)
                DCP_ROW2(1, 0) DCP_ROW2(2, 1) DCP_ROW2(3, 0) DCP_ROW2(4, 1) DCP_ROW2(0, 0)
            }
            if (j <= L) DCP_ROW2(1, 1)
            if (j <= L) DCP_ROW2(2, 0)
            if (j <= L) DCP_ROW2(3, 1)
            if (j <= L) DCP_ROW2(4, 0)
            if (j <= L) DCP_ROW2(0, 1)
            if (j <= L) DCP_ROW2(1, 0)
            if (j <= L) DCP_ROW2(2, 1)
            if (j <= L) DCP_ROW2(3, 0)
            if (j <= L) DCP_ROW2(4, 1)
#undef DCP_ROW2
#undef DCP_E3
        }
        else
        {
        unsigned w = base_at(words, 0);
        load_row<R, STAGED>(em_base, ldk, lane_boff, eN_tab, eI_tab, w, em, em[2], em[3], em[4], eN, eI, stg, swd);

#define DCP_ROW(PH)                                                            \
    {                                                                          \
        w = ((w << 2) | base_at(words, j)) & 1023u;                            \
        o = dp_row<R, W, PH>(s, t, em, em[2], em[3], em[4], eN, eI, sp, xEB, xc, wave, lane, gen, exact_e, [&]() { \
            load_row<R, STAGED>(em_base, ldk, lane_boff, eN_tab, eI_tab, w, em, em[2], em[3], em[4], eN, eI, stg, swd); \
        }, sink);                                                              \
        ++j;                                                                   \
    }
        while (j + 4 <= L)
        {
            DCP_ROW(1) DCP_ROW(2) DCP_ROW(3) DCP_ROW(4) DCP_ROW(0)
        }
        if (j <= L) DCP_ROW(1)
        if (j <= L) DCP_ROW(2)
        if (j <= L) DCP_ROW(3)
        if (j <= L) DCP_ROW(4)
        }
#undef DCP_ROW

        float const C = __builtin_bit_cast(float, __builtin_amdgcn_readlane(__builtin_bit_cast(int, o.X), 2));
        float const nul = __builtin_bit_cast(float, __builtin_amdgcn_readlane(__builtin_bit_cast(int, o.X), 3));
        float const alt = fmaxf(o.E + xt[DCP_X_ET], C + xt[DCP_X_CT]);
        if constexpr (TRACE)
        {
            if (threadIdx.x == (W == 1 ? wave * 64u : 0u)) a.trace_alt[task] = alt;
            continue;
        }
        if (threadIdx.x == (W == 1 ? wave * 64u : 0u))
        {
            size_t const oi = (size_t)q * a.nprof_total + pm.pidx;
            if (a.out_null) a.out_null[oi] = nul;
            if (a.out_alt) a.out_alt[oi] = alt;
            if (dcp_lrt_hit(nul, alt, a.lrt_threshold))
            {
                unsigned const h = atomicAdd(a.nhits, 1u);
                if (h < a.hit_cap)
                    a.hits[h] = dcp_hit{a.q_base + q, pm.pidx, nul, alt};
            }
        }
    }
    if (!pair_mode) break;
    }
}

template <int K>
__global__ __launch_bounds__(256, 3) void viterbi_mp_kernel(dcp_scan_args a)
{
    constexpr int R = 4;
    constexpr unsigned PL = 64u / K;
    constexpr unsigned MAXLD = 4u * 72u + 16u;
    constexpr int STAGED = 20;
    __shared__ __attribute__((aligned(16))) float stage_mem[STAGED * MAXLD];
    unsigned const lane = threadIdx.x & 63u;
    unsigned const wave = __builtin_amdgcn_readfirstlane(threadIdx.x >> 6);
    unsigned const nblk = gridDim.x;
    unsigned const vblk = (blockIdx.x & 7u) * (nblk >> 3) + (blockIdx.x >> 3);
    unsigned const bpp = (a.nseqs + 3u) / 4u;
    if (vblk >= a.nprof * bpp) return;
    unsigned const g_rel = vblk / bpp;
    unsigned const qi = (vblk - g_rel * bpp) * 4u + wave;
    bool const has_q = qi < a.nseqs;
    unsigned const q = __builtin_amdgcn_readfirstlane(has_q ? qi : 0u);
    dcp_mp_group const *gp = a.mp_groups + (a.first_prof + g_rel);
    unsigned const ldk = __builtin_amdgcn_readfirstlane(gp->ldk);
    unsigned const nparts = __builtin_amdgcn_readfirstlane(gp->nparts);
    float const *__restrict__ em_base = a.emis_match + gp->emis_off;
    {
        float4 const *__restrict__ src = reinterpret_cast<float4 const *>(em_base);
        float4 *dst = reinterpret_cast<float4 *>(stage_mem);
        for (unsigned i = threadIdx.x; i < (unsigned)STAGED * (ldk >> 2); i += 256u)
            dst[i] = src[i];
        __syncthreads();
    }
    if (!has_q) return;
    float const *const stg = stage_mem;
    float const ni = neg_inf();
    unsigned const part = lane / PL, pl = lane % PL;
    unsigned const M = gp->core_size[part];
    unsigned const node0 = pl * R;
    unsigned const lane_off = gp->col0[part] + (node0 < M ? node0 : ((M + 3u) & ~3u));
    Trans<R> t;
    {
        float const *__restrict__ tb = a.trans8 + gp->trans_off + lane_off;
        VecLoad<R>::ld(tb + (size_t)DCP_T_ENTRY * ldk, t.ent);
        VecLoad<R>::ld(tb + (size_t)DCP_T_MM * ldk, t.mm);
        VecLoad<R>::ld(tb + (size_t)DCP_T_IM * ldk, t.im);
        VecLoad<R>::ld(tb + (size_t)DCP_T_DM * ldk, t.dm);
        VecLoad<R>::ld(tb + (size_t)DCP_T_MD * ldk, t.md);
        VecLoad<R>::ld(tb + (size_t)DCP_T_DD * ldk, t.dd);
        VecLoad<R>::ld(tb + (size_t)DCP_T_MI * ldk, t.mi);
        VecLoad<R>::ld(tb + (size_t)DCP_T_II * ldk, t.ii);
    }
    float2 const *__restrict__ in_tab = reinterpret_cast<float2 const *>(a.mp_in) + gp->in_off;
    unsigned part_boff = part * 8u;

    unsigned const L = a.seq_len[q];
    cu32 *words = as_const(a.seq_words + a.seq_woff[q]);
    cfloat *xt = as_const(a.xtrans + (size_t)q * DCP_XSTRIDE);
    unsigned const x = lane & 3u;
    LaneSpecial sp;
    sp.a = x == 1u ? xt[DCP_X_EJ] : x == 2u ? xt[DCP_X_EC] : ni;
    sp.b = x == 0u ? xt[DCP_X_NN] : x == 1u ? xt[DCP_X_JJ] : x == 2u ? xt[DCP_X_CC] : xt[DCP_X_RR];
    sp.c = x == 0u ? xt[DCP_X_NB] : x == 1u ? xt[DCP_X_JB] : ni;
    float const xEB = xt[DCP_X_EB];
// ... 687 lines not shown
                    b[x2] * b[x3] * s1(C, x1));
    }
    if (code < 340)
    {
        int v = (int)code - 84;
        int x[4] = {v >> 6, (v >> 4) & 3, (v >> 2) & 3, v & 3};
        double one = b[x[0]] * c3(C, x[1], x[2], x[3]) + b[x[1]] * c3(C, x[0], x[2], x[3]) +
                     b[x[2]] * c3(C, x[0], x[1], x[3]) + b[x[3]] * c3(C, x[0], x[1], x[2]);
        double two = 0;
#pragma unroll
        for (int i = 0; i < 4; ++i)
#pragma unroll
            for (int j = i + 1; j < 4; ++j)
            {
                int r[2], n = 0;
#pragma unroll
                for (int k = 0; k < 4; ++k)
                    if (k != i && k != j) r[n++] = x[k];
                two += b[x[i]] * b[x[j]] * s2(C, r[0], r[1]);
            }
        return e * f2 * f / 2.0 * one + e2 * e * f / 9.0 * two;
    }
    {
        int v = (int)code - 340;
        int x[5] = {v >> 8, (v >> 6) & 3, (v >> 4) & 3, (v >> 2) & 3, v & 3};
        double s = 0;
#pragma unroll
        for (int i = 0; i < 5; ++i)
#pragma unroll
            for (int j = i + 1; j < 5; ++j)
            {
                int r[3], n = 0;
#pragma unroll
                for (int k = 0; k < 5; ++k)
                    if (k != i && k != j) r[n++] = x[k];
                s += b[x[i]] * b[x[j]] * c3(C, r[0], r[1], r[2]);
            }
        return e2 * f2 / 10.0 * s;
    }
}
}

__global__ __launch_bounds__(256) void expand_tables_kernel(dcp_expand_args a)
{
    __shared__ double lin[64][DCP_NDIST + 1];
    dcp_expand_tile const tile = a.tiles[blockIdx.x];
    float const *__restrict__ dist = a.dists + (size_t)tile.dist_row * DCP_NDIST;
    unsigned const nk = tile.ncols;
    for (unsigned i = threadIdx.x; i < 64u * DCP_NDIST; i += 256u)
    {
        unsigned k = i / DCP_NDIST, c = i - k * DCP_NDIST;
        lin[k][c] = k < nk ? exp((double)dist[(size_t)k * DCP_NDIST + c]) : 0.0;
    }
    __syncthreads();
    unsigned const k = threadIdx.x & 63u;
    double const e = k < nk ? (double)a.eps[tile.dist_row + k] : 0.0, f = 1.0 - e;
    size_t col_off = (size_t)k * tile.ld_col;
    unsigned ld_code = tile.ld_code;
    if (tile.kt)
    {
        unsigned const node = tile.col0 + k, kt = tile.kt;
        col_off = ((size_t)(node / kt) * (kt / 4u) + (node % kt) / 4u) * (size_t)DCP_NCODES * 4u + (node & 3u);
        ld_code = 4u;
    }
    float *__restrict__ out = a.out + tile.out_off + col_off;
    for (unsigned code = threadIdx.x >> 6; code < DCP_NCODES; code += 4u)
    {
        float v = -__builtin_inff();
        if (k < nk) v = (float)log(frame_prob(&lin[k][0], &lin[k][4], e, f, code));
        if (k < tile.nstore) out[(size_t)code * ld_code] = v;
    }
}

extern "C" void dcp_launch_expand(dcp_expand_args const *a, unsigned ntiles,
                                  void *stream)
{
    hipLaunchKernelGGL(expand_tables_kernel, dim3(ntiles), dim3(256), 0,
                       (hipStream_t)stream, *a);
}

template <int R, int W, int STG, bool PF = false>
static void launch_rs(dcp_scan_args const *a, unsigned nblocks, unsigned threads, hipStream_t s, unsigned pad_lds = 0)
{
    hipLaunchKernelGGL((viterbi_rowsweep_kernel<R, W, STG, PF>), dim3(nblocks), dim3(threads), pad_lds, s, *a);
}

extern "C" unsigned dcp_rowsweep_tasks_per_block(int W) { return W == 1 ? 4u : 1u; }

extern "C" unsigned dcp_rowsweep_max_block_waves(int R, int W, int stg)
{
    if (W != 1) return stg == 0 ? 1u : 0u;
    if (stg == 0) return 4u;
    if (stg == 20) return R >= 1 && R <= 8 ? (unsigned)std::min(rs_block_threads(R, 1, 20, false), rs_block_threads(R, 1, 20, true)) / 64u : 0u;
    if (stg == 84) return R >= 1 && R <= 7 ? (unsigned)rs_block_threads(R, 1, 84) / 64u : 0u;
    return 0u;
}
extern "C" unsigned dcp_rowsweep_stage_bytes(int R, int stg) { return (unsigned)stg * (64u * (unsigned)R + (R <= 2 ? 8u : 0u)) * 4u; }

extern "C" int dcp_launch_rowsweep_grid(int R, int W, dcp_scan_args const *a, int stg, unsigned bw, void *stream,
                                        unsigned pad_lds, int prefetch2)
{
    hipStream_t s = (hipStream_t)stream;
    unsigned const maxw = dcp_rowsweep_max_block_waves(R, W, stg);
    if (maxw == 0u || (stg > 0 && (bw == 0u || bw > maxw))) return -1;
    uint64_t nb;
    if (stg > 0) nb = (uint64_t)a->nprof * ((a->nchunks + bw - 1u) / bw);
    else nb = ((uint64_t)a->nprof * a->nchunks + dcp_rowsweep_tasks_per_block(W) - 1u) / dcp_rowsweep_tasks_per_block(W);
    nb = (nb + 7u) / 8u * 8u;
    if (nb > 0x7fffffffull) return -2;
    unsigned const nblocks = (unsigned)nb;
    {
        unsigned const used = dcp_rowsweep_stage_bytes(R, stg) + 1024u;
        pad_lds = used >= 160u * 1024u ? 0u : std::min(pad_lds, 160u * 1024u - used);
    }
#define DCP_CASE_S(r, g)                                                       \
    if (R == r && W == 1 && stg == g)                                          \
    {                                                                          \
        if (prefetch2) launch_rs<r, 1, g, true>(a, nblocks, 64u * bw, s, pad_lds); \
        else launch_rs<r, 1, g, false>(a, nblocks, 64u * bw, s, pad_lds);      \
        return 0;                                                              \
    }
    DCP_CASE_S(1, 20) DCP_CASE_S(2, 20) DCP_CASE_S(3, 20) DCP_CASE_S(4, 20) DCP_CASE_S(5, 20) DCP_CASE_S(6, 20)
    DCP_CASE_S(7, 20) DCP_CASE_S(8, 20)
    DCP_CASE_S(1, 84) DCP_CASE_S(2, 84) DCP_CASE_S(3, 84) DCP_CASE_S(4, 84) DCP_CASE_S(5, 84) DCP_CASE_S(6, 84)
    DCP_CASE_S(7, 84)
#undef DCP_CASE_S
    if (stg != 0) return -1;
    return dcp_launch_rowsweep(R, W, a, nblocks, stream);
}

extern "C" int dcp_launch_mp(int K, dcp_scan_args const *a, void *stream)
{
    uint64_t nb = (uint64_t)a->nprof * ((a->nseqs + 3u) / 4u);
    nb = (nb + 7u) / 8u * 8u;
    if (nb > 0x7fffffffull) return -2;
    if (K == 4) hipLaunchKernelGGL((viterbi_mp_kernel<4>), dim3((unsigned)nb), dim3(256), 0, (hipStream_t)stream, *a);
    else if (K == 2) hipLaunchKernelGGL((viterbi_mp_kernel<2>), dim3((unsigned)nb), dim3(256), 0, (hipStream_t)stream, *a);
    else return -1;
    return 0;
}
extern "C" void dcp_launch_mp_in(dcp_mp_group const *groups, unsigned ngroups, unsigned n_first, unsigned k_first, unsigned k_rest,
                                 float const *emis_insert, float const *emis_null, float *out, void *stream)
{
    hipLaunchKernelGGL(mp_in_kernel, dim3(ngroups), dim3(256), 0, (hipStream_t)stream, groups, n_first, k_first, k_rest,
                       emis_insert, emis_null, out);
}

extern "C" unsigned dcp_segsweep_blocks(unsigned nprof, unsigned nq) { return (nprof * ((nq + 3u) / 4u) + 7u) / 8u * 8u; }
extern "C" int dcp_launch_segsweep(int R, dcp_scan_args const *a, unsigned nblocks, void *stream)
{
#define DCP_CASE_G(r)                                                                                          \
    if (R == r)                                                                                                \
    {                                                                                                          \
        hipLaunchKernelGGL((viterbi_segment_kernel<r>), dim3(nblocks), dim3(256), 0, (hipStream_t)stream, *a); \
        return 0;                                                                                              \
    }
    DCP_CASE_G(5) DCP_CASE_G(6) DCP_CASE_G(7) DCP_CASE_G(8)
#undef DCP_CASE_G
    return -1;
}

extern "C" int dcp_launch_trace_forward(int R, int W, dcp_scan_args const *a, unsigned nblocks, void *stream)
{
#define DCP_CASE_T(r, w)                                                                                        \
    if (R == r && W == w)                                                                                       \
    {                                                                                                           \
// ... 26 lines not shown
```

### deciphon-old_amd/csrc/dcp_qlane.hip

```cpp
#include "dcp_kernels.h"

#include <hip/hip_runtime.h>
#include <type_traits>

namespace
{
constexpr int NC = DCP_NCODES;

#ifndef DCP_QLANE_RECOMPUTE_B
#define DCP_QLANE_RECOMPUTE_B 1
#endif
constexpr bool kRecomputeB = DCP_QLANE_RECOMPUTE_B != 0;
#ifndef DCP_QLANE_WD
#define DCP_QLANE_WD 5
#endif
constexpr unsigned kWD = DCP_QLANE_WD;
constexpr unsigned kPlanes = kRecomputeB ? 3u : 4u;
#ifndef DCP_QLANE_DIAG
#define DCP_QLANE_DIAG 0
#endif

#ifndef DCP_QL_WPLANE
#define DCP_QL_WPLANE 1
#endif
// ... 33 lines not shown

struct SweepOut
{
    float E, C, Rn;
};

template <int G> struct TileTrans
{
    float ent[4 * G], mi[4 * G], ii[4 * G];
    float mm[4 * G + 1], im[4 * G + 1], dm[4 * G + 1], md[4 * G + 1], dd[4 * G + 1];
};

template <int G> __device__ __forceinline__ void load_tile_trans(TileTrans<G> &t, cfloat *tt)
{
    constexpr int KT = 4 * G;
#pragma unroll
    for (int k = 0; k < KT; ++k)
    {
        t.ent[k] = tt[k * 8 + DCP_T_ENTRY];
        t.mi[k] = tt[k * 8 + DCP_T_MI];
        t.ii[k] = tt[k * 8 + DCP_T_II];
    }
#pragma unroll
    for (int k = 1; k <= KT; ++k)
    {
        t.mm[k] = tt[k * 8 + DCP_T_MM];
        t.im[k] = tt[k * 8 + DCP_T_IM];
        t.dm[k] = tt[k * 8 + DCP_T_DM];
        t.md[k] = tt[k * 8 + DCP_T_MD];
        t.dd[k] = tt[k * 8 + DCP_T_DD];
    }
    t.mm[0] = t.im[0] = t.dm[0] = t.md[0] = t.dd[0] = 0.0f;
}

struct RowIn
{
    float4 e0[5];
    float eI[5], eN[5];
};

template <int G, bool ROWS>
__device__ __forceinline__ void stage_tile_image(float *tabM, dcp_qlane_args const &a, dcp_ql_prof const &pm, unsigned t,
                                                 unsigned first, unsigned stride)
{
    constexpr unsigned N4 = (unsigned)(G * NC);
    float4 *dst = reinterpret_cast<float4 *>(tabM);
    if constexpr (!ROWS)
    {
        float4 const *__restrict__ src = reinterpret_cast<float4 const *>(a.emis_tiles + pm.tile_off + (size_t)t * (N4 * 4u));
        for (unsigned i = first; i < N4; i += stride)
            dst[i] = src[i];
    }
    else
    {
        float const *__restrict__ rows = a.emis_tiles + pm.tile_off + t * (4u * (unsigned)G);
        unsigned const ldk = pm.ldk, M = pm.core_size;
        for (unsigned i = first; i < N4; i += stride)
        {
            unsigned const grp = i / (unsigned)NC, code = i - grp * (unsigned)NC;
            float4 v = make_float4(ninf(), ninf(), ninf(), ninf());
            if (t * (4u * (unsigned)G) + grp * 4u < M)
                v = *reinterpret_cast<float4 const *>(rows + (size_t)code * ldk + grp * 4u);
            dst[i] = v;
        }
    }
}

__device__ __forceinline__ float ld_off(float const *base, unsigned boff)
{
    return *reinterpret_cast<float const *>(reinterpret_cast<char const *>(base) + boff);
}
typedef uint32_t const __attribute__((address_space(1))) *gu32_ptr;
typedef uint16_t const __attribute__((address_space(1))) *gu16_ptr;
typedef char const __attribute__((address_space(1))) *gchar_ptr;
__device__ __forceinline__ void st_off(float *base, unsigned boff, float v)
{
    *reinterpret_cast<float *>(reinterpret_cast<char *>(base) + boff) = v;
}

struct Ring
{
    float B[5], Xm[5], Xd[5], Em[5];
};

enum
{
    IO_HBM = 1,
    IO_LDS = 2
};
constexpr unsigned kRD = 16;
constexpr unsigned kRLanes = 256;
constexpr unsigned kRingPlaneBytes = kRD * kRLanes * 4u;
#ifndef DCP_Q2_SKEW
#define DCP_Q2_SKEW 4
#endif
#ifndef DCP_Q2_HYST
#define DCP_Q2_HYST 1
#endif
#ifndef DCP_Q2_SLEEP
#define DCP_Q2_SLEEP 2
#endif
#ifndef DCP_Q2_PRIO
#define DCP_Q2_PRIO 0
#endif
#ifndef DCP_Q2_STAGEMAP
#define DCP_Q2_STAGEMAP 1
#endif
constexpr unsigned kRingSkew = DCP_Q2_SKEW;
constexpr unsigned kRingHyst = DCP_Q2_HYST;
typedef float __attribute__((address_space(3))) lds_float;
typedef unsigned __attribute__((address_space(3))) lds_uint;

typedef char __attribute__((address_space(3))) lds_char;

struct LdsLink
{
    lds_char *base;
    unsigned my_flag;
    unsigned peer_flag;
    unsigned seen;
};
constexpr unsigned kL2ImageBytes = 2u * 1364u * 16u;
constexpr unsigned kL2TabIN = kL2ImageBytes;
constexpr unsigned kL2TabINBytes = 1364u * 16u;
constexpr unsigned kL2Base1 = 32768u;
constexpr unsigned kL2Tab1 = 65536u;
constexpr unsigned kL2FlagP = kL2Tab1 + kL2ImageBytes;
constexpr unsigned kL2FlagC = kL2FlagP + kRLanes * 4u;
constexpr unsigned kL2Task = kL2FlagC + kRLanes * 4u;
constexpr unsigned kL2Abort = kL2Task + 4u;
constexpr unsigned kL2Err = kL2Task + 8u;
constexpr unsigned kL2Ring = 7u * kRingPlaneBytes;
constexpr unsigned kL2Bytes = kL2Ring + 3u * kRingPlaneBytes;
static_assert(kL2TabIN + kL2TabINBytes <= kL2Tab1, "LDS layout: the table ends in front of image 1");
static_assert(kL2Err + 8u <= kL2Ring && (kL2Err & 7u) == 0u, "LDS layout: flags and words end in front of the ring");
static_assert(kL2Bytes == 160u * 1024u, "LDS layout: all of the CU's LDS");
static_assert(kL2Base1 <= kL2TabIN && kL2Base1 <= kL2Tab1, "stage 1's base is below everything it gathers from");
static_assert(0u + (340u + 1364u) * 16u + 16u <= 65535u && kL2TabIN + 340u * 16u + 8u <= 65535u, "stage 0: DS immediates are 16 bits");
static_assert(kL2Tab1 - kL2Base1 + (340u + 1364u) * 16u + 16u <= 65535u && kL2TabIN - kL2Base1 + 340u * 16u + 8u <= 65535u,
              "stage 1: DS immediates are 16 bits");
static_assert((kL2Ring & (kRingPlaneBytes - 1u)) == 0u, "ring slots are addressed by OR");
static_assert(kRD >= 12u, "a shorter ring can deadlock the two stages (five-row hand-shake groups)");

__device__ __forceinline__ void compiler_fence() { asm volatile("" ::: "memory"); }
#define DCP_ISA_MARK(name) asm volatile("; " name ::: "memory")
__device__ __forceinline__ unsigned flag_load(lds_uint *flag)
{
    return __hip_atomic_load(flag, __ATOMIC_RELAXED, __HIP_MEMORY_SCOPE_WORKGROUP);
}
__device__ __forceinline__ void flag_store(lds_uint *flag, unsigned v)
{
    __hip_atomic_store(flag, v, __ATOMIC_RELAXED, __HIP_MEMORY_SCOPE_WORKGROUP);
}
#ifndef DCP_Q2_BOUND
#define DCP_Q2_BOUND 1
#endif
constexpr unsigned kRingSpinBound = 1u << 23;
constexpr unsigned kRingPoison = 0x7fffff00u;
__device__ __forceinline__ unsigned ring_wait(LdsLink const &lk, unsigned need)
{
    lds_uint *flag = (lds_uint *)(lk.base + lk.peer_flag);
    unsigned v = __builtin_amdgcn_readfirstlane(flag_load(flag));
#if DCP_Q2_BOUND
    unsigned spins = 0;
#pragma nounroll
    while (v < need)
    {
        __builtin_amdgcn_s_sleep(DCP_Q2_SLEEP);
        v = __builtin_amdgcn_readfirstlane(flag_load(flag));
        if (__builtin_expect(++spins == kRingSpinBound, 0))
        {
            typedef unsigned __attribute__((address_space(1))) *gerr_ptr;
            gerr_ptr const err = *(gerr_ptr __attribute__((address_space(3))) *)(lk.base + kL2Err);
            __hip_atomic_store(err, 1u, __ATOMIC_RELAXED, __HIP_MEMORY_SCOPE_AGENT);
            flag_store((lds_uint *)(lk.base + kL2Abort), 1u);
            flag_store(flag, kRingPoison);
            v = kRingPoison;
            __builtin_amdgcn_s_waitcnt(0x0070);
        }
    }
#else
    while (v < need)
    {
        __builtin_amdgcn_s_sleep(DCP_Q2_SLEEP);
        v = __builtin_amdgcn_readfirstlane(flag_load(flag));
    }
#endif
    DCP_ISA_MARK("DCP_RING_ACQUIRED");
    return v;
}
__device__ __forceinline__ float ring_ld(LdsLink const &lk, unsigned rowoff, unsigned plane)
{
    return *(lds_float *)(lk.base + ((rowoff & (kRingPlaneBytes - 1u)) | kL2Ring) + plane * kRingPlaneBytes);
}
__device__ __forceinline__ void ring_st(LdsLink const &lk, unsigned rowoff, unsigned plane, float v)
{
    *(lds_float *)(lk.base + ((rowoff & (kRingPlaneBytes - 1u)) | kL2Ring) + plane * kRingPlaneBytes) = v;
}
__device__ __forceinline__ void ring_publish(LdsLink const &lk, unsigned rowoff, unsigned row)
{
    flag_store((lds_uint *)(lk.base + lk.my_flag + (rowoff & (kRLanes * 4u - 1u))), row);
}

template <bool FIRST>
__device__ __forceinline__ void ring_fetch_x(Ring &r, int slot, float const *pXm, float const *pXd,
                                             float const *pEm, unsigned off)
{
    if constexpr (!FIRST)
    {
        r.Xm[slot] = ld_off(pXm, off);
        r.Xd[slot] = ld_off(pXd, off);
        r.Em[slot] = ld_off(pEm, off);
    }
}
template <bool FIRST>
__device__ __forceinline__ void ring_fetch_b(Ring &r, int slot, float const *pB, unsigned off)
{
    if constexpr (!kRecomputeB && !FIRST) r.B[slot] = ld_off(pB, off);
}
template <bool FIRST>
__device__ __forceinline__ void ring_fetch(Ring &r, int slot, float const *pB, float const *pXm,
                                           float const *pXd, float const *pEm, unsigned off)
{
    ring_fetch_x<FIRST>(r, slot, pXm, pXd, pEm, off);
    ring_fetch_b<FIRST>(r, slot, pB, off);
}

struct GatherOff
{
    unsigned a[5];
};
template <unsigned BASE> struct GatherMasks
{
    unsigned base, m[4];
    __device__ __forceinline__ GatherMasks()
    {
        static_assert((BASE & 0x3fffu) == 0u, "the base must not overlap the window's 14 bits");
        base = BASE;
        if constexpr (BASE != 0u) asm volatile("" : "+s"(base));
#pragma unroll
        for (int l = 0; l < 4; ++l)
            m[l] = (((1u << (2 * l + 2)) - 1u) << 4) | base;
    }
};
template <unsigned BASE> __device__ __forceinline__ GatherOff gather_off(unsigned w, GatherMasks<BASE> const &gm)
{
    unsigned const wp = (DCP_QLANE_DIAG & 1) ? 0u : w;
    unsigned const w16 = kWPlane ? (BASE != 0u ? (wp | gm.base) : wp) : ((w << 4) | gm.base);
    GatherOff g;
#pragma unroll
    for (int l = 0; l < 4; ++l)
        g.a[l] = w16 & gm.m[l];
    if constexpr (kWPlane && BASE == 0u && !(DCP_QLANE_DIAG & 1)) asm volatile("v_mov_b32 %0, %1" : "=v"(g.a[4]) : "v"(w16));
    else g.a[4] = w16;
    return g;
}
template <int GROUP> __device__ __forceinline__ float4 gather_match(float const *tabM, GatherOff const &g, int l)
{
    constexpr unsigned first[5] = {0u, 4u, 20u, 84u, 340u};
    return *reinterpret_cast<float4 const *>(reinterpret_cast<char const *>(tabM) +
                                             (g.a[l] + (first[l] + (unsigned)GROUP * NC) * 16u));
}

template <int G, bool FIRST, bool LAST, bool IN16>
__device__ __forceinline__ void ql_fetch(RowIn &in, float const *tabM, float2 const *tabIN, GatherOff const &g)
{
    constexpr unsigned first[5] = {0u, 4u, 20u, 84u, 340u};
#pragma unroll
    for (int l = 0; l < 5; ++l)
    {
        in.e0[l] = gather_match<0>(tabM, g, l);
        float2 const v = *reinterpret_cast<float2 const *>(
            reinterpret_cast<char const *>(tabIN) + (IN16 ? g.a[l] + first[l] * 16u : (g.a[l] >> 1) + first[l] * 8u));
        in.eI[l] = v.x;
        in.eN[l] = v.y;
    }
}

template <int R> __device__ __forceinline__ float comp(float4 const &v)
{
    return R == 0 ? v.x : R == 1 ? v.y : R == 2 ? v.z : v.w;
}

template <int G, bool FIRST, bool LAST, int PH, int NT, int D, int IN = IO_HBM, int OUT = IO_HBM, unsigned TBASE = 0u,
          bool IN16 = kIn16, int NV = 4 * G>
__device__ __forceinline__ void ql_row(QState<G> &s, TileTrans<G> const &tr, float const *tabM,
                                       float2 const *tabIN, GatherOff &go,
                                       unsigned wn, RowIn &in, Ring &ring, float *pB, float *pXm,
                                       float *pXd, float *pEm, unsigned &off, LaneXt const &xt,
                                       bool live, bool at_end, bool &dirty, SweepOut &o,
                                       LdsLink const &lk, unsigned jrow, GatherMasks<TBASE> const &gm
#if DCP_QLANE_DIAG & 4
                                       , unsigned &off2, unsigned din
#endif
                                       )
{
    constexpr int KT = 4 * G;
    static_assert(LAST || NV == 4 * G, "only a last tile has pad nodes to leave out");
    static_assert(NV % 2 == 0 && NV >= 2 && NV <= 4 * G, "E is folded over node pairs");
    constexpr bool kGroup1 = G > 1 && NV > 4;
    constexpr int s1 = (PH + 4) % 5, s2 = (PH + 3) % 5, s3 = (PH + 2) % 5, s4 = (PH + 1) % 5, s5 = PH;
    float const ni = ninf();

    static_assert(G <= 2, "gather_match<GROUP> is instantiated for groups 0 and 1");
    float4 e[G > 1 ? G - 1 : 1][5];
    if constexpr (kGroup1)
    {
#pragma unroll
        for (int l = 0; l < 5; ++l)
            e[0][l] = gather_match<1>(tabM, go, l);
    }

    {
        constexpr int per_row = ((FIRST || IN != IO_HBM) ? 0 : 3) + ((LAST || OUT != IO_HBM) ? 0 : 3) +
                                ((!kRecomputeB && !FIRST) ? 1 : 0) + ((!kRecomputeB && FIRST) ? 1 : 0) + 1;
        constexpr int vm = ((D < (int)kWD ? D : (int)kWD) - 1) * per_row;
        constexpr int lgkm = kGroup1 ? 5 : 0;
        __builtin_amdgcn_s_waitcnt((vm & 15) | ((vm >> 4) << 14) | (7 << 4) | (lgkm << 8));
    }
    __builtin_amdgcn_sched_barrier(0);
    float Xm = ni, Xd = ni, E = ni, Bj = ring.B[PH];
    if constexpr (!FIRST)
    {
        Xm = ring.Xm[PH];
        Xd = ring.Xd[PH];
        E = ring.Em[PH];
    }
    float eI[5], eN[5];
#pragma unroll
    for (int l = 0; l < 5; ++l)
    {
        eI[l] = in.eI[l];
        eN[l] = in.eN[l];
    }

    if constexpr (FIRST || kRecomputeB)
    {
        float const N = mx5(s.PN[s1] + eN[0], s.PN[s2] + eN[1], s.PN[s3] + eN[2],
                            s.PN[s4] + eN[3], s.PN[s5] + eN[4]);
        s.PN[PH] = N + xt.NN;
        Bj = N + xt.NB;
        if constexpr (FIRST)
        {
            float const Rn = mx5(s.PR[s1] + eN[0], s.PR[s2] + eN[1], s.PR[s3] + eN[2],
                                 s.PR[s4] + eN[3], s.PR[s5] + eN[4]);
            s.PR[PH] = Rn + xt.RR;
            o.Rn = at_end ? Rn : o.Rn;
            if constexpr (!kRecomputeB) st_off(pB, off, Bj);
        }
    }

    float pm = ni, pi = ni, pd = ni;
    float m_even = ni;
    auto node = [&](int k, float e0, float e1, float e2, float e3, float e4) {
        float const m = mx5(s.P[s1][k] + e0, s.P[s2][k] + e1, s.P[s3][k] + e2, s.P[s4][k] + e3,
                            s.P[s5][k] + e4);
        float const iv = mx5(s.Q[s1][k] + eI[0], s.Q[s2][k] + eI[1], s.Q[s3][k] + eI[2],
                             s.Q[s4][k] + eI[3], s.Q[s5][k] + eI[4]);
        float d, pin;
        if (k == 0)
        {
            d = Xd;
            pin = Xm;
        }
        else
        {
            d = fmaxf(pm + tr.md[k], pd + tr.dd[k]);
            pin = mx3(pm + tr.mm[k], pi + tr.im[k], pd + tr.dm[k]);
        }
        if constexpr (kEM)
        {
            if (k & 1) E = mx3(E, m_even, m);
            else m_even = m;
        }
        else E = mx3(E, m, d);
        s.P[PH][k] = fmaxf(Bj + tr.ent[k], pin);
        s.Q[PH][k] = fmaxf(m + tr.mi[k], iv + tr.ii[k]);
        pm = m, pi = iv, pd = d;
    };

    node(0, in.e0[0].x, in.e0[1].x, in.e0[2].x, in.e0[3].x, in.e0[4].x);
    node(1, in.e0[0].y, in.e0[1].y, in.e0[2].y, in.e0[3].y, in.e0[4].y);
    if constexpr (NV > 2)
    {
        node(2, in.e0[0].z, in.e0[1].z, in.e0[2].z, in.e0[3].z, in.e0[4].z);
        node(3, in.e0[0].w, in.e0[1].w, in.e0[2].w, in.e0[3].w, in.e0[4].w);
    }

    if constexpr (!FIRST && IN == IO_HBM)
    {
        asm volatile("" : "+v"(off) : "v"(E));
#if DCP_QLANE_DIAG & 4
        ring_fetch_x<FIRST>(ring, (PH + D) % 5, pXm + din, pXd + din, pEm + din, off);
#else
        ring_fetch_x<FIRST>(ring, (PH + D) % 5, pXm + D * NT, pXd + D * NT, pEm + D * NT, off);
#endif
    }

    __builtin_amdgcn_s_waitcnt(0xC07F | (0 << 8));
    go = gather_off<TBASE>(wn, gm);
    ql_fetch<G, FIRST, LAST, IN16>(in, tabM, tabIN, go);
    if constexpr (!FIRST && IN == IO_LDS)
    {
        constexpr int sl = (PH + 1) % 5;
        DCP_ISA_MARK("DCP_RING_TAKE");
        unsigned const nxt = off + kRLanes * 4u;
        ring.Xm[sl] = ring_ld(lk, nxt, 0);
        ring.Xd[sl] = ring_ld(lk, nxt, 1);
        ring.Em[sl] = ring_ld(lk, nxt, 2);
        DCP_ISA_MARK("DCP_RING_TAKEN");
        ring_publish(lk, off, jrow + 1u);
        DCP_ISA_MARK("DCP_RING_TAKE_END");
    }

#pragma unroll
    for (int g = 1; g < G; ++g)
    {
        float4 const *eg = e[g - 1];
        if (4 * g + 0 < NV)
        {
            node(4 * g + 0, eg[0].x, eg[1].x, eg[2].x, eg[3].x, eg[4].x);
            node(4 * g + 1, eg[0].y, eg[1].y, eg[2].y, eg[3].y, eg[4].y);
        }
        if (4 * g + 2 < NV)
        {
            node(4 * g + 2, eg[0].z, eg[1].z, eg[2].z, eg[3].z, eg[4].z);
            node(4 * g + 3, eg[0].w, eg[1].w, eg[2].w, eg[3].w, eg[4].w);
        }
    }

    if constexpr (!kRecomputeB && !FIRST)
    {
        asm volatile("" : "+v"(off) : "v"(pm));
        ring_fetch_b<FIRST>(ring, (PH + D) % 5, pB + D * NT, off);
    }

    if constexpr (!LAST)
    {
        float const oXm = mx3(pm + tr.mm[KT], pi + tr.im[KT], pd + tr.dm[KT]);
        float const oXd = fmaxf(pm + tr.md[KT], pd + tr.dd[KT]);
        if constexpr (OUT == IO_LDS)
        {
            DCP_ISA_MARK("DCP_RING_DATA");
            ring_st(lk, off, 0, oXm);
            ring_st(lk, off, 1, oXd);
            ring_st(lk, off, 2, E);
            DCP_ISA_MARK("DCP_RING_FLAG");
            ring_publish(lk, off, jrow);
            DCP_ISA_MARK("DCP_RING_DATA_END");
        }
        else
        {
#if DCP_QLANE_DIAG & 4
            unsigned const offw = off2;
#else
            unsigned const offw = off;
#endif
            st_off(pXm, offw, oXm);
            st_off(pXd, offw, oXd);
            st_off(pEm, offw, E);
        }
    }
    else
    {
        float const J = mx5(s.PJ[s1] + eN[0], s.PJ[s2] + eN[1], s.PJ[s3] + eN[2], s.PJ[s4] + eN[3],
                            s.PJ[s5] + eN[4]);
        float const C = mx5(s.PC[s1] + eN[0], s.PC[s2] + eN[1], s.PC[s3] + eN[2], s.PC[s4] + eN[3],
                            s.PC[s5] + eN[4]);
        float const B1 = fmaxf(E + xt.EB, J + xt.JB);
        dirty = dirty || (live && B1 > Bj);
        s.PJ[PH] = fmaxf(E + xt.EJ, J + xt.JJ);
        s.PC[PH] = fmaxf(E + xt.EC, C + xt.CC);
        o.E = at_end ? E : o.E;
        o.C = at_end ? C : o.C;
    }
}

template <int G, bool FIRST, bool LAST, int NT, int D, int IN = IO_HBM, int OUT = IO_HBM, unsigned TBASE = 0u,
          bool IN16 = kIn16, int NV = 4 * G>
__device__ __forceinline__ void ql_sweep(cfloat *tt, float const *tabM, float2 const *tabIN,
                                         uint32_t const *__restrict__ wordsT, unsigned rowbase,
                                         unsigned L, unsigned Lwave, bool active, float *sc,
                                         size_t plane, unsigned tid, LaneXt const &xt, bool &dirty,
                                         SweepOut &o, LdsLink lk
#if DCP_QLANE_DIAG & 4
                                         , unsigned tile_odd
#endif
                                         )
{
    constexpr int KT = 4 * G;
#if DCP_QLANE_DIAG & 4
    unsigned const rowstep = tile_odd ? 0u : (unsigned)NT;
    unsigned const rowstep_out = tile_odd ? (unsigned)NT : 0u;
    unsigned const din = (unsigned)D * rowstep;
    unsigned off2 = tid * 4u;
#else
    constexpr unsigned rowstep = (DCP_QLANE_DIAG & 2) ? 0u : (unsigned)NT;
#endif
    float const ni = ninf();
    TileTrans<G> tr;
    load_tile_trans<G>(tr, tt);
    QState<G> s;
#pragma unroll
    for (int h = 0; h < 5; ++h)
    {
#pragma unroll
        for (int k = 0; k < KT; ++k)
            s.P[h][k] = ni, s.Q[h][k] = ni;
        s.PN[h] = ni, s.PR[h] = ni, s.PJ[h] = ni, s.PC[h] = ni;
    }
    {
        float const B0 = 0.0f + xt.SB;
#pragma unroll
        for (int k = 0; k < KT; ++k)
            s.P[0][k] = B0 + tr.ent[k];
        s.PN[0] = 0.0f + xt.SN;
        s.PR[0] = 0.0f;
    }
    float *pXm = sc, *pXd = sc + plane, *pEm = sc + 2 * plane, *pB = sc + (kRecomputeB ? 0 : 3) * plane;
    unsigned off = (rowbase * (unsigned)NT + tid) * 4u;

    unsigned j = 1;
    static_assert(kWPlane, "the packed-word sequence planes are gone (round 4): a slot's groups are addressed by plane row");
    typedef uint16_t wq_t;
    wq_t wq[5];
    unsigned w;
    unsigned lane2 = tid * 2u;
    gu16_ptr const wpl = (gu16_ptr)wordsT + (size_t)rowbase * (unsigned)NT;
    asm volatile("" : "+v"(lane2));
    {
        w = wpl[NT + tid];
#pragma unroll
        for (int r = 2; r < 7; ++r)
            wq[r % 5] = wpl[r * NT + tid];
        __builtin_amdgcn_sched_barrier(0);
        __builtin_amdgcn_s_waitcnt(0x0F70);
    }
    RowIn in;
    Ring ring;
#pragma unroll
    for (int l = 0; l < 5; ++l)
    {
        in.e0[l] = float4{ni, ni, ni, ni}, in.eI[l] = ni, in.eN[l] = ni;
        ring.B[l] = ring.Xm[l] = ring.Xd[l] = ring.Em[l] = ni;
    }
    GatherMasks<TBASE> const gm;
    GatherOff go = gather_off<TBASE>(w, gm);
    ql_fetch<G, FIRST, LAST, IN16>(in, tabM, tabIN, go);
    if constexpr (!FIRST && IN == IO_LDS)
    {
        static_assert(NT == (int)kRLanes, "the ring's row stride is the scratch planes' row stride");
        unsigned const need0 = rowbase + (Lwave < kRingSkew ? Lwave : kRingSkew);
        lk.seen = ring_wait(lk, need0);
        DCP_ISA_MARK("DCP_RING_TAKE");
        ring.Xm[1] = ring_ld(lk, off, 0);
        ring.Xd[1] = ring_ld(lk, off, 1);
        ring.Em[1] = ring_ld(lk, off, 2);
        DCP_ISA_MARK("DCP_RING_TAKEN");
        ring_publish(lk, off, rowbase + 1u);
        DCP_ISA_MARK("DCP_RING_TAKE_END");
    }
    else
    {
        lk.seen = 0u;
#pragma unroll
        for (int r = 0; r < D; ++r)
            ring_fetch<(FIRST || IN != IO_HBM)>(ring, (r + 1) % 5, pB, pXm, pXd, pEm, off + (unsigned)r * rowstep * 4u);
    }

#if DCP_QLANE_DIAG & 8
#ifndef DCP_QLANE_DIAG_ROWS
#define DCP_QLANE_DIAG_ROWS 256u
#endif
#define QL_DIAG8_WRAP off &= (DCP_QLANE_DIAG_ROWS * (unsigned)NT * 4u - 1u);
#else
#define QL_DIAG8_WRAP
#endif
#if DCP_QLANE_DIAG & 4
#define QL_DIAG4_ARGS , off2, din
#define QL_DIAG4_STEP off2 += rowstep_out * 4u;
#else
#define QL_DIAG4_ARGS
#define QL_DIAG4_STEP
#endif
#define QL_ROW(PH)                                                                         \
    {                                                                                      \
                                                 \
        unsigned const pos = j + 1u;                                                       \
        ql_row<G, FIRST, LAST, PH, NT, D, IN, OUT, TBASE, IN16, NV>(s, tr, tabM, tabIN, go,          \
                                   (unsigned)wq[(PH + 1) % 5], in, ring, pB, pXm,                    \
                                   pXd, pEm, off, xt, active && j <= L, active && j == L,  \
                                   dirty, o, lk, rowbase + j, gm QL_DIAG4_ARGS);           \
        {    \
             \
             \
             \
             \
            gu16_ptr wrow = wpl + (pos + 5u) * (unsigned)NT;                                     \
            asm volatile("" : "+s"(wrow));                                                   \
            asm volatile("" : "+v"(lane2));  \
            wq[(PH + 1) % 5] = *(gu16_ptr)((gchar_ptr)wrow + lane2);                          \
        }                                                                                    \
        off += rowstep * 4u;                                                                     \
        QL_DIAG8_WRAP                                                                            \
        QL_DIAG4_STEP                                                                            \
        ++j;                                                                               \
             \
             \
             \
        __builtin_amdgcn_sched_barrier(6);                                                 \
    }
    auto ring_sync = [&](unsigned n) {
        if constexpr (!FIRST && IN == IO_LDS)
        {
            unsigned const need = rowbase + (j + n < Lwave ? j + n : Lwave);
            if (lk.seen < need) lk.seen = ring_wait(lk, need + kRingHyst < rowbase + Lwave ? need + kRingHyst : rowbase + Lwave);
        }
        if constexpr (!LAST && OUT == IO_LDS)
        {
            unsigned const last = rowbase + j + n - 1u;
            if (last > lk.seen + kRD) lk.seen = ring_wait(lk, last - kRD + kRingHyst);
        }
    };
    while (j + 4 <= Lwave)
    {
        ring_sync(5u);
        QL_ROW(1) QL_ROW(2) QL_ROW(3) QL_ROW(4) QL_ROW(0)
    }
    ring_sync(4u);
    if (j <= Lwave) QL_ROW(1)
    if (j <= Lwave) QL_ROW(2)
    if (j <= Lwave) QL_ROW(3)
    if (j <= Lwave) QL_ROW(4)
#undef QL_ROW
}

template <bool IN16>
__device__ __forceinline__ void fill_tab_in(float *tab, float const *__restrict__ gi, float const *__restrict__ gn, unsigned t,
                                            unsigned nthreads)
{
    for (unsigned i = t; i < (unsigned)NC; i += nthreads)
    {
        if constexpr (IN16) *reinterpret_cast<float4 *>(tab + 4u * i) = float4{gi[i], gn[i], 0.0f, 0.0f};
        else *reinterpret_cast<float2 *>(tab + 2u * i) = float2{gi[i], gn[i]};
    }
}

typedef dcp_ql_group const __attribute__((address_space(4))) cgroup;
typedef uint32_t const __attribute__((address_space(4))) cu32;

struct GroupLane
{
    unsigned q, L, Lwave, rowbase;
    bool has;
    LaneXt xt;
};
__device__ __forceinline__ void load_group(dcp_qlane_args const &a, unsigned gi, unsigned lane, GroupLane &g)
{
    cgroup *gd = (cgroup *)(unsigned long long)(a.groups + gi);
    unsigned const qfirst = gd->qfirst, nq = gd->nq;
    g.rowbase = gd->rowbase;
    g.has = lane < nq;
    g.q = g.has ? a.qorder[qfirst + lane] : 0u;
    g.L = g.has ? a.seq_len[g.q] : 0u;
    g.Lwave = gd->lmax;
    float const *__restrict__ x = a.xtrans + (size_t)g.q * DCP_XSTRIDE;
    g.xt.RR = x[DCP_X_RR], g.xt.SB = x[DCP_X_SB], g.xt.SN = x[DCP_X_SN], g.xt.NN = x[DCP_X_NN];
    g.xt.NB = x[DCP_X_NB], g.xt.ET = x[DCP_X_ET], g.xt.EC = x[DCP_X_EC], g.xt.CC = x[DCP_X_CC];
    g.xt.CT = x[DCP_X_CT], g.xt.EB = x[DCP_X_EB], g.xt.EJ = x[DCP_X_EJ], g.xt.JJ = x[DCP_X_JJ];
    g.xt.JB = x[DCP_X_JB];
    __builtin_amdgcn_s_waitcnt(0x0F70);
    __builtin_amdgcn_sched_barrier(0);
}
__device__ __forceinline__ unsigned park_off(GroupLane const &g, unsigned NT, unsigned col)
{
    return ((g.rowbase + g.Lwave + 8u) * NT + col) * 4u;
}

__device__ __forceinline__ void ql_publish(dcp_qlane_args const &a, dcp_ql_prof const &pm, unsigned q, float nul, float alt,
                                           bool redo)
{
    if (redo)
    {
        unsigned const cls = pm.cls;
        unsigned const i = atomicAdd(a.redo_n + cls, 1u);
        if (i < a.redo_cap[cls]) a.redo[a.redo_base[cls] + i] = dcp_pair{q, pm.rs_slot};
        else *a.redo_overflow = 1u;
        return;
    }
    size_t const oi = (size_t)q * a.nprof_total + pm.pidx;
    if (a.out_null) a.out_null[oi] = nul;
    if (a.out_alt) a.out_alt[oi] = alt;
    if (dcp_lrt_hit(nul, alt, a.lrt_threshold))
    {
        unsigned const h = atomicAdd(a.nhits, 1u);
        if (h < a.hit_cap) a.hits[h] = dcp_hit{a.q_base + q, pm.pidx, nul, alt};
    }
}

}

template <int G, int NT, int D, bool ROWS = false>
__global__ __launch_bounds__(NT, NT / 128) void viterbi_qlane_kernel(dcp_qlane_args a)
{
    constexpr int KT = 4 * G;
    constexpr int TAB_FLOATS = G * NC * 4;
    __shared__ __attribute__((aligned(16))) float lds[TAB_FLOATS + (kIn16 ? 4 : 2) * NC];
    __shared__ unsigned s_task;
    float *tabM = lds;
    float2 *tabIN = reinterpret_cast<float2 *>(lds + TAB_FLOATS);
    unsigned const tid = threadIdx.x;
    size_t const plane = (size_t)a.plane_rows * (unsigned)NT;
    float *const sc = a.scratch + (size_t)blockIdx.x * kPlanes * plane;
    constexpr unsigned SLOTS = (unsigned)NT / 64u;

    for (;;)
    {
        if (tid == 0) s_task = atomicAdd(a.task_counter, 1u);
        __syncthreads();
        unsigned const task = __builtin_amdgcn_readfirstlane(s_task);
        __syncthreads();
        if (task >= a.ntasks) break;
        unsigned const slot = a.nprof - 1u - task / a.nqblocks;
        unsigned const qb = task % a.nqblocks;
        dcp_ql_prof const pm = a.profs[slot];
        unsigned const T = pm.ntiles;
        unsigned const sidx = __builtin_amdgcn_readfirstlane(qb * SLOTS + (tid >> 6));
        cu32 *sf = (cu32 *)(unsigned long long)a.slot_first;
        unsigned const g0 = sf[sidx], g1 = sf[sidx + 1u];
        uint32_t const *__restrict__ wordsT = a.words_t + __builtin_amdgcn_readfirstlane(a.wt_off[qb]);

        {
            float const *__restrict__ gi = a.emis_insert + (size_t)pm.pidx * NC;
            float const *__restrict__ gn = a.emis_null + (size_t)pm.pidx * NC;
            fill_tab_in<kIn16>(lds + TAB_FLOATS, gi, gn, tid, (unsigned)NT);
        }

        GroupLane g;
        bool const single = g1 - g0 == 1u;
        bool t_loaded = false;
        for (unsigned t = 0; t < T; ++t)
        {
            __syncthreads();
            stage_tile_image<G, ROWS>(tabM, a, pm, t, tid, (unsigned)NT);
            __syncthreads();
            cfloat *tt = as_const(a.ttrans + pm.ttrans_off + (size_t)t * (KT + 1) * 8);
            bool const first = t == 0, last = t + 1 == T;
            for (unsigned gi = g0; gi < g1; ++gi)
            {
                if (!(single && t_loaded)) load_group(a, gi, tid & 63u, g);
                t_loaded = true;
                if (g.Lwave == 0u) continue;
                SweepOut o{ninf(), ninf(), ninf()};
                bool dirty = false;
#if DCP_QLANE_DIAG & 4
#define QL_DIAG4_TILE , (t & 1u)
#else
#define QL_DIAG4_TILE
#endif
#define QL_SWEEP(F, L_)                                                                          \
    ql_sweep<G, F, L_, NT, D>(tt, tabM, tabIN, wordsT, g.rowbase, g.L, g.Lwave, g.has, sc, plane, tid, g.xt, dirty, o, LdsLink{} QL_DIAG4_TILE)
                if (first && last) QL_SWEEP(true, true);
                else if (first) QL_SWEEP(true, false);
                else if (last) QL_SWEEP(false, true);
                else QL_SWEEP(false, false);
#undef QL_SWEEP
                unsigned const po = park_off(g, (unsigned)NT, tid);
                if (first && !last) st_off(sc, po, o.Rn);
                if (last && g.has)
                {
                    float const nul = first ? o.Rn : ld_off(sc, po);
                    ql_publish(a, pm, g.q, nul, fmaxf(o.E + g.xt.ET, o.C + g.xt.CT), dirty || (kEM && pm.needs_exact_e));
                }
            }
        }
    }
}

template <int G, int D, bool ROWS = false>
__global__ __launch_bounds__(512, 2) void viterbi_qlane2_kernel(dcp_qlane_args a)
{
    constexpr int NT = (int)kRLanes;
    constexpr int KT = 4 * G;
    __shared__ __attribute__((aligned(16))) float lds[kL2Bytes / 4u];
    unsigned const wv = threadIdx.x >> 6;
#if DCP_Q2_STAGEMAP == 0
    unsigned const stage = __builtin_amdgcn_readfirstlane(wv & 1u);
    unsigned const tid = ((wv >> 1) << 6) | (threadIdx.x & 63u);
#else
    unsigned const stage = __builtin_amdgcn_readfirstlane(wv >> 2);
    unsigned const tid = threadIdx.x & 255u;
#endif
    unsigned *const s_task_p = reinterpret_cast<unsigned *>(lds + kL2Task / 4u);
    float *const tabM = lds + (stage ? kL2Tab1 / 4u : 0u);
    size_t const plane = (size_t)a.plane_rows * (unsigned)NT;
    float *const sc = a.scratch + (size_t)blockIdx.x * kPlanes * plane;
    constexpr unsigned SLOTS = (unsigned)NT / 64u;

#if DCP_Q2_PRIO == 1
    if (stage == 1u) __builtin_amdgcn_s_setprio(1);
#elif DCP_Q2_PRIO == 2
    if (stage == 0u) __builtin_amdgcn_s_setprio(1);
#endif
    LdsLink lk;
    lk.base = (lds_char *)lds;
    lk.my_flag = stage == 0u ? kL2FlagP : kL2FlagC;
    lk.peer_flag = (stage == 0u ? kL2FlagC : kL2FlagP) + (tid & ~63u) * 4u;
    lk.seen = 0u;
    if (threadIdx.x == 0) *(unsigned **)(lds + kL2Err / 4u) = a.ring_error;
    unsigned *const s_abort_p = reinterpret_cast<unsigned *>(lds + kL2Abort / 4u);

    for (;;)
    {
        if (threadIdx.x == 0)
        {
            unsigned const failed = __hip_atomic_load(a.ring_error, __ATOMIC_RELAXED, __HIP_MEMORY_SCOPE_AGENT);
            unsigned const next = atomicAdd(a.task_counter, 1u);
            *s_task_p = failed ? 0xffffffffu : next;
            *s_abort_p = 0u;
        }
        __syncthreads();
        unsigned const task = __builtin_amdgcn_readfirstlane(*s_task_p);
        __syncthreads();
        if (task >= a.ntasks) break;
        unsigned const slot = a.nprof - 1u - task / a.nqblocks;
        unsigned const qb = task % a.nqblocks;
        dcp_ql_prof const pm = a.profs[slot];
        unsigned const T = pm.ntiles;
        unsigned const sidx = __builtin_amdgcn_readfirstlane(qb * SLOTS + (tid >> 6));
        cu32 *sf = (cu32 *)(unsigned long long)a.slot_first;
        unsigned const g0 = sf[sidx], g1 = sf[sidx + 1u];
        uint32_t const *__restrict__ wordsT = a.words_t + __builtin_amdgcn_readfirstlane(a.wt_off[qb]);
        {
            float const *__restrict__ gi = a.emis_insert + (size_t)pm.pidx * NC;
            float const *__restrict__ gn = a.emis_null + (size_t)pm.pidx * NC;
            fill_tab_in<true>(lds + kL2TabIN / 4u, gi, gn, threadIdx.x, 512u);
        }
        bool const stalled = a.ring_stall != 0u && task == 0u && stage == 0u;

        unsigned const nsteps = (T + 1u) / 2u;
        unsigned const final_stage = (T - 1u) & 1u;
        GroupLane g;
        bool const single = g1 - g0 == 1u;
        bool t_loaded = false;
        for (unsigned st = 0; st < nsteps; ++st)
        {
            unsigned const t = 2u * st + stage;
            bool const mine = t < T;
            __syncthreads();
            if (mine) stage_tile_image<G, ROWS>(tabM, a, pm, t, tid, (unsigned)NT);
            flag_store((lds_uint *)(lk.base + lk.my_flag + tid * 4u), 0u);
            __syncthreads();
            if (!mine || (stalled && st == 0u) || __builtin_amdgcn_readfirstlane(*s_abort_p) != 0u) continue;
            cfloat *tt = as_const(a.ttrans + pm.ttrans_off + (size_t)t * (KT + 1) * 8);
            bool const first = t == 0u, last = t + 1u == T;
#if DCP_QLANE_DIAG & 4
#error "the two-stage kernel has no DIAG=4 build"
#endif
            for (unsigned gi = g0; gi < g1; ++gi)
            {
                if (!(single && t_loaded)) load_group(a, gi, tid & 63u, g);
                t_loaded = true;
                if (g.Lwave == 0u) continue;
                SweepOut o{ninf(), ninf(), ninf()};
                bool dirty = false;
#define QL2_SWEEP_NV(F, L_, IN_, OUT_, TB_, IMG_, NV_)                                                    \
    ql_sweep<G, F, L_, NT, D, IN_, OUT_, TB_, true, NV_>(tt, lds + ((IMG_) - (TB_)) / 4u,                  \
                                              reinterpret_cast<float2 const *>(lds + (kL2TabIN - (TB_)) / 4u), \
                                              wordsT, g.rowbase, g.L, g.Lwave, g.has, sc, plane, tid, g.xt, dirty, o, lk)
#define QL2_SWEEP(F, L_, IN_, OUT_, TB_, IMG_) QL2_SWEEP_NV(F, L_, IN_, OUT_, TB_, IMG_, KT)
#define QL2_SWEEP_LAST(IN_, TB_, IMG_)                                                                    \
    switch ((pm.core_size - t * (unsigned)KT + 1u) & ~1u)                                                 \
    {                                                                                                     \
    case 2u: QL2_SWEEP_NV(false, true, IN_, IO_HBM, TB_, IMG_, 2); break;                                 \
    case 4u: QL2_SWEEP_NV(false, true, IN_, IO_HBM, TB_, IMG_, 4); break;                                 \
    case 6u: QL2_SWEEP_NV(false, true, IN_, IO_HBM, TB_, IMG_, 6); break;                                 \
    default: QL2_SWEEP_NV(false, true, IN_, IO_HBM, TB_, IMG_, KT); break;                                \
    }
                static_assert(KT == 8, "QL2_SWEEP_LAST names the node counts of an 8-node tile");
                if (stage == 0u)
                {
                    if (first && last) QL2_SWEEP(true, true, IO_HBM, IO_HBM, 0u, 0u);
                    else if (first) QL2_SWEEP(true, false, IO_HBM, IO_LDS, 0u, 0u);
                    else if (last) QL2_SWEEP_LAST(IO_HBM, 0u, 0u)
                    else QL2_SWEEP(false, false, IO_HBM, IO_LDS, 0u, 0u);
                }
                else
                {
                    if (last) QL2_SWEEP_LAST(IO_LDS, kL2Base1, kL2Tab1)
                    else QL2_SWEEP(false, false, IO_LDS, IO_HBM, kL2Base1, kL2Tab1);
                }
#undef QL2_SWEEP_LAST
#undef QL2_SWEEP
#undef QL2_SWEEP_NV
                unsigned const po = park_off(g, (unsigned)NT, tid);
                if (first) st_off(sc, po, o.Rn);
                if (last)
                {
                    st_off(sc + plane, po, fmaxf(o.E + g.xt.ET, o.C + g.xt.CT));
                    st_off(sc + 2 * plane, po, dirty ? 1.0f : 0.0f);
                }
            }
        }
        __syncthreads();

        if (stage != final_stage) continue;
        for (unsigned gi = g0; gi < g1; ++gi)
        {
            cgroup *gd = (cgroup *)(unsigned long long)(a.groups + gi);
            GroupLane ge;
            ge.rowbase = gd->rowbase, ge.Lwave = gd->lmax;
            if (ge.Lwave == 0u || (tid & 63u) >= gd->nq) continue;
            unsigned const q = a.qorder[gd->qfirst + (tid & 63u)];
            unsigned const po = park_off(ge, (unsigned)NT, tid);
            float const nul = ld_off(sc, po), alt = ld_off(sc + plane, po);
            bool const dirty = ld_off(sc + 2 * plane, po) != 0.0f;
            ql_publish(a, pm, q, nul, alt, dirty || (kEM && pm.needs_exact_e));
        }
    }
}

template <int G, int D, bool ROWS = false>
__global__ __launch_bounds__(192, 1) void viterbi_qlane_w3_kernel(dcp_qlane_args a)
{
    constexpr int NT = 64;
    constexpr int KT = 4 * G;
    constexpr int TAB_FLOATS = G * NC * 4;
    constexpr int SLICE = TAB_FLOATS + 2 * NC;
    __shared__ __attribute__((aligned(16))) float lds[3 * SLICE];
    unsigned const wv = __builtin_amdgcn_readfirstlane(threadIdx.x >> 6);
    unsigned const tid = threadIdx.x & 63u;
    float *const tabM = lds + wv * SLICE;
    float2 *const tabIN = reinterpret_cast<float2 *>(tabM + TAB_FLOATS);
    size_t const plane = (size_t)a.plane_rows * (unsigned)NT;
    float *const sc = a.scratch + ((size_t)blockIdx.x * 3u + wv) * kPlanes * plane;

    for (;;)
    {
        unsigned t0 = 0;
        if (tid == 0) t0 = atomicAdd(a.task_counter, 1u);
        unsigned const task = __builtin_amdgcn_readfirstlane(t0);
        if (task >= a.ntasks) break;
        unsigned const slot = a.nprof - 1u - task / a.nqblocks;
        unsigned const qb = task % a.nqblocks;
        dcp_ql_prof const pm = a.profs[slot];
        unsigned const T = pm.ntiles;
        cu32 *sf = (cu32 *)(unsigned long long)a.slot_first;
        unsigned const g0 = sf[qb], g1 = sf[qb + 1u];
        uint32_t const *__restrict__ wordsT = a.words_t + __builtin_amdgcn_readfirstlane(a.wt_off[qb]);
        {
            float const *__restrict__ gi = a.emis_insert + (size_t)pm.pidx * NC;
            float const *__restrict__ gn = a.emis_null + (size_t)pm.pidx * NC;
            for (unsigned i = tid; i < (unsigned)NC; i += (unsigned)NT)
                tabIN[i] = float2{gi[i], gn[i]};
        }
        GroupLane g;
        bool const single = g1 - g0 == 1u;
        bool t_loaded = false;
        for (unsigned t = 0; t < T; ++t)
        {
            stage_tile_image<G, ROWS>(tabM, a, pm, t, tid, (unsigned)NT);
            compiler_fence();
            cfloat *tt = as_const(a.ttrans + pm.ttrans_off + (size_t)t * (KT + 1) * 8);
            bool const first = t == 0, last = t + 1 == T;
            for (unsigned gi = g0; gi < g1; ++gi)
            {
                if (!(single && t_loaded)) load_group(a, gi, tid, g);
                t_loaded = true;
                if (g.Lwave == 0u) continue;
                SweepOut o{ninf(), ninf(), ninf()};
                bool dirty = false;
#define QLW_SWEEP(F, L_)                                                                                  \
    ql_sweep<G, F, L_, NT, D, IO_HBM, IO_HBM, 0u, false>(tt, tabM, tabIN, wordsT, g.rowbase, g.L, g.Lwave, g.has, sc, plane, tid, g.xt, dirty, o, LdsLink{})
                if (first && last) QLW_SWEEP(true, true);
                else if (first) QLW_SWEEP(true, false);
                else if (last) QLW_SWEEP(false, true);
                else QLW_SWEEP(false, false);
#undef QLW_SWEEP
                unsigned const po = park_off(g, (unsigned)NT, tid);
                if (first && !last) st_off(sc, po, o.Rn);
                if (last && g.has)
                {
                    float const nul = first ? o.Rn : ld_off(sc, po);
                    ql_publish(a, pm, g.q, nul, fmaxf(o.E + g.xt.ET, o.C + g.xt.CT), dirty || (kEM && pm.needs_exact_e));
                }
            }
            compiler_fence();
        }
    }
}

template <int NT>
__global__ __launch_bounds__(NT) void transpose_words_kernel(dcp_qlane_args a)
{
    unsigned const qb = blockIdx.x, tid = threadIdx.x;
    unsigned const rows = (a.wt_off[qb + 1] - a.wt_off[qb]) * 2u / (unsigned)NT;
    uint16_t *dst = reinterpret_cast<uint16_t *>(a.words_t + a.wt_off[qb]);
    unsigned const sidx = qb * ((unsigned)NT / 64u) + (tid >> 6);
    unsigned const g0 = a.slot_first[sidx], g1 = a.slot_first[sidx + 1u];
    unsigned r = 0;
    for (unsigned gi = g0; gi < g1; ++gi)
    {
        dcp_ql_group const g = a.groups[gi];
        bool const has = (tid & 63u) < g.nq;
        unsigned const q = has ? a.qorder[g.qfirst + (tid & 63u)] : 0u;
        uint32_t const *__restrict__ src = a.seq_words + a.seq_woff[q];
        unsigned const len = has ? a.seq_len[q] : 0u;
        for (; r < g.rowbase; ++r)
            dst[r * (unsigned)NT + tid] = 0;
        unsigned w = 0, word = 0;
        unsigned const gr = g.lmax + 10u;
        for (unsigned k = 0; k < gr && r < rows; ++k, ++r)
        {
            if (k >= 1u)
            {
                unsigned const pos = k - 1u;
                if ((pos & 15u) == 0u) word = pos < len ? src[pos >> 4] : 0u;
                w = ((w << 2) | ((pos < len ? word >> ((pos & 15u) * 2u) : 0u) & 3u)) & 1023u;
            }
            dst[r * (unsigned)NT + tid] = (uint16_t)(w << 4);
        }
    }
    for (; r < rows; ++r)
        dst[r * (unsigned)NT + tid] = 0;
}

template <int G, int NT, int D>
static void launch_ql(dcp_qlane_args const *a, unsigned nblocks, hipStream_t s)
{
    if (a->tiles_from_rows) hipLaunchKernelGGL((viterbi_qlane_kernel<G, NT, D, true>), dim3(nblocks), dim3(NT), 0, s, *a);
    else hipLaunchKernelGGL((viterbi_qlane_kernel<G, NT, D>), dim3(nblocks), dim3(NT), 0, s, *a);
}

#ifndef DCP_QLANE_NT
#define DCP_QLANE_NT 256
#endif
#ifndef DCP_QLANE_D
#define DCP_QLANE_D 3
#endif
extern "C" unsigned dcp_qlane_block_size(void) { return DCP_QLANE_NT; }
extern "C" unsigned dcp_qlane_tile_nodes(void) { return 8u; }
extern "C" unsigned dcp_qlane_scratch_planes(void) { return kPlanes; }
extern "C" unsigned dcp_qlane_diag_build(void) { return DCP_QLANE_DIAG; }
extern "C" unsigned dcp_qlane_group_rows(unsigned lmax) { return (lmax + 11u) & ~1u; }
extern "C" unsigned dcp_qlane_window_planes(void) { return kWPlane ? 1u : 0u; }
extern "C" unsigned dcp_qlane_exact_e_by_redo(void) { return kEM ? 1u : 0u; }

extern "C" int dcp_launch_qlane_transpose(dcp_qlane_args const *a, unsigned nt, void *stream)
{
    if (nt == 64) hipLaunchKernelGGL((transpose_words_kernel<64>), dim3(a->nqblocks), dim3(64), 0, (hipStream_t)stream, *a);
    else if (nt == DCP_QLANE_NT)
        hipLaunchKernelGGL((transpose_words_kernel<DCP_QLANE_NT>), dim3(a->nqblocks), dim3(DCP_QLANE_NT), 0, (hipStream_t)stream, *a);
    else return 1;
    return 0;
}

extern "C" unsigned dcp_qlane2_lds_bytes(void) { return kL2Bytes; }

extern "C" int dcp_launch_qlane_w3(dcp_qlane_args const *a, unsigned nblocks, void *stream)
{
    if (a->tiles_from_rows)
        hipLaunchKernelGGL((viterbi_qlane_w3_kernel<2, DCP_QLANE_D, true>), dim3(nblocks), dim3(192), 0, (hipStream_t)stream, *a);
    else hipLaunchKernelGGL((viterbi_qlane_w3_kernel<2, DCP_QLANE_D>), dim3(nblocks), dim3(192), 0, (hipStream_t)stream, *a);
    return 0;
}

extern "C" int dcp_launch_qlane2(dcp_qlane_args const *a, unsigned nblocks, void *stream)
{
    if (a->tiles_from_rows)
        hipLaunchKernelGGL((viterbi_qlane2_kernel<2, DCP_QLANE_D, true>), dim3(nblocks), dim3(512), 0, (hipStream_t)stream, *a);
    else hipLaunchKernelGGL((viterbi_qlane2_kernel<2, DCP_QLANE_D>), dim3(nblocks), dim3(512), 0, (hipStream_t)stream, *a);
    return 0;
}

extern "C" int dcp_launch_qlane(dcp_qlane_args const *a, unsigned nblocks, unsigned nt, void *stream)
{
    if (nt == DCP_QLANE_NT) launch_ql<2, DCP_QLANE_NT, DCP_QLANE_D>(a, nblocks, (hipStream_t)stream);
    else return 1;
    return 0;
}
```

### deciphon-old_amd/csrc/dcp_test_hooks.h

```cpp
#ifndef DCP_TEST_HOOKS_H
#define DCP_TEST_HOOKS_H

#include "dcp_host.h"

#define DCP_RS_PATH_NONE 0u
#define DCP_RS_PATH_PLAIN 1u
#define DCP_RS_PATH_MP 2u
#define DCP_RS_PATH_SEGMENTED 3u
#define DCP_RS_PLAN_WORDS 9u
#define DCP_PL_SCAN_PAIRS 1u
#define DCP_PL_QLANE_REDO 2u
#define DCP_PL_SEG_REDO 3u
#define DCP_PL_WORDS 7u

#ifdef DCP_TEST_HOOKS
extern "C" {
int dcp_gpu_test_last_rowsweep_plan(dcp_gpu_ctx *, unsigned *out, unsigned cap, unsigned *nwords);
int dcp_gpu_test_last_pair_launches(dcp_gpu_ctx *, unsigned *out, unsigned cap, unsigned *nwords);
int dcp_gpu_test_set_forward_waves(dcp_gpu_ctx *, unsigned nwaves);
int dcp_gpu_test_set_dense_round(dcp_gpu_ctx *, unsigned npairs);
int dcp_gpu_test_set_forward_scale_band(dcp_gpu_ctx *, unsigned bits);
int dcp_gpu_test_set_posterior_budget(dcp_gpu_ctx *, unsigned long long bytes);
int dcp_gpu_test_set_mea_budget(dcp_gpu_ctx *, unsigned long long bytes);
}
#endif

#endif
```

Baseline: 1458.

## Resume redo rowsweep from recorded suffix instead of recomputing whole pair

The two-stage query-lane scan now records the first dirty row for pairs that need an exact redo, and saves a suffix record holding the X-state and the known partial E values from that row onward. The one-wavefront pair-mode rowsweep redo kernel then starts at that row using the saved state, so it skips the rows already computed correctly. This trims redo work but adds scratch traffic, atomics and a new buffer sized from sequence length, plus extra kernel template variants that raise code complexity and register pressure.

New measurement: 1459, median of 2. Within noise of the previous version (+0.1%).

```diff
diff --git a/deciphon-old_amd/__init__.py b/deciphon-old_amd/__init__.py
--- a/deciphon-old_amd/__init__.py
+++ b/deciphon-old_amd/__init__.py
@@ -307,6 +307,8 @@
         sig["dcp_gpu_test_set_forward_scale_band"] = (I, [P, U])
         sig["dcp_gpu_test_set_posterior_budget"] = (I, [P, C.c_ulonglong])
         sig["dcp_gpu_test_set_mea_budget"] = (I, [P, C.c_ulonglong])
+        sig["dcp_gpu_test_set_suffix_cap"] = (I, [P, C.c_ulonglong])
+        sig["dcp_gpu_test_last_suffix_pairs"] = (I, [P, P, U, C.POINTER(U), C.POINTER(U)])
     for name, (res, args) in sig.items():
         fn = getattr(lib, name)
         fn.restype = res
@@ -1395,6 +1397,19 @@
 
     def test_set_redo_cap(self, cap):
         self._check(self._lib.dcp_gpu_test_set_redo_cap(self._c, int(cap)))
+
+    def test_set_suffix_cap(self, floats):
+        self._check(self._lib.dcp_gpu_test_set_suffix_cap(self._c, int(floats)))
+
+    def test_suffix_pairs(self):
+        n, without = C.c_uint(0), C.c_uint(0)
+        rc = self._lib.dcp_gpu_test_last_suffix_pairs(self._c, None, 0, C.byref(n), C.byref(without))
+        if rc != RC_ENOMEM:
+            self._check(rc)
+        w = np.zeros(3 * n.value, np.uint32)
+        if n.value:
+            self._check(self._lib.dcp_gpu_test_last_suffix_pairs(self._c, w.ctypes.data, len(w), C.byref(n), C.byref(without)))
+        return w.reshape(-1, 3), int(without.value)
 
     def test_set_ring_stall(self, on):
         self._check(self._lib.dcp_gpu_test_set_ring_stall(self._c, int(bool(on))))
diff --git a/deciphon-old_amd/csrc/dcp_gpu.hip b/deciphon-old_amd/csrc/dcp_gpu.hip
--- a/deciphon-old_amd/csrc/dcp_gpu.hip
+++ b/deciphon-old_amd/csrc/dcp_gpu.hip
@@ -154,6 +154,8 @@
     uint64_t pair_class_cells[DCP_MAX_CLASSES] = {0}, pair_class_bytes[DCP_MAX_CLASSES] = {0};
     bool redo_pending = false, redo_pending64 = false, ring_check_pending = false;
 #ifdef DCP_TEST_HOOKS
+    bool sfx = false;
+    unsigned redo_base[DCP_MAX_CLASSES] = {0}, redo_cap[DCP_MAX_CLASSES] = {0};
     struct RowsweepClassPlan
     {
         unsigned path = 0;
@@ -223,6 +225,10 @@
     DevBuf<unsigned> d_task_counter;
     DevBuf<dcp_pair> d_redo;
     DevBuf<unsigned> d_redo_n;
+    DevBuf<float> d_sfx_buf;
+    DevBuf<unsigned long long> d_sfx_n;
+    DevBuf<uint32_t> d_redo_sfx;
+    uint64_t sfx_cap_forced = 0;
     unsigned qorder_q0 = ~0u, qorder_q1 = ~0u, qorder_lmax = 0;
     unsigned num_cus = 0;
     unsigned qorder_nt = 0;
@@ -2666,6 +2672,27 @@
             redo_grid[k] = (unsigned)((g + 7) / 8 * 8);
         }
         HIP_TRY(c, c->d_redo.reserve((size_t)tot));
+        if (two_stage)
+        {
+            uint64_t const pairs = (uint64_t)a.nseqs * c->nprof;
+            unsigned lmax = 0;
+            for (unsigned q = a.q_base; q < a.q_base + a.nseqs; ++q)
+                lmax = std::max<unsigned>(lmax, c->seq_len[q]);
+            uint64_t cap = std::max<uint64_t>((pairs + 31u) / 32u * ((uint64_t)lmax + 16u), (uint64_t)1 << 20);
+            if (c->sfx_cap_forced) cap = c->sfx_cap_forced;
+            cap = std::min<uint64_t>(cap, 0xffffffffull);
+            HIP_TRY(c, c->d_sfx_buf.reserve((size_t)cap));
+            HIP_TRY(c, c->d_sfx_n.reserve(1));
+            HIP_TRY(c, c->d_redo_sfx.reserve((size_t)tot));
+            HIP_TRY(c, hipMemsetAsync(c->d_sfx_n.p, 0, sizeof(unsigned long long), c->stream));
+            HIP_TRY(c, hipMemsetAsync(c->d_redo_sfx.p, 0xff, (size_t)tot * sizeof(uint32_t), c->stream));
+            qa.redo_sfx = c->d_redo_sfx.p;
+            qa.sfx_buf = c->d_sfx_buf.p;
+            qa.sfx_n = c->d_sfx_n.p;
+            qa.sfx_cap = cap;
+            for (int k = 0; k < kNumClasses; ++k)
+                if (kClasses[k].W == 1) qa.sfx_classes |= 1u << k;
+        }
     }
     HIP_TRY(c, c->d_redo_n.reserve(DCP_MAX_CLASSES + 2));
     HIP_TRY(c, hipMemsetAsync(c->d_redo_n.p, 0, (DCP_MAX_CLASSES + 2) * sizeof(unsigned), c->stream));
@@ -2701,13 +2728,22 @@
         a.first_prof = 0;
         a.nprof = c->nprof;
         SizeClass const sc = kClasses[k];
+        bool const sfx_k = qa.redo_sfx != nullptr && ((qa.sfx_classes >> k) & 1u) != 0u;
+        a.pair_sfx = sfx_k ? qa.redo_sfx + qa.redo_base[k] : nullptr;
+        a.sfx_buf = sfx_k ? qa.sfx_buf : nullptr;
         if (dcp_launch_rowsweep(sc.R, sc.W, &a, redo_grid[k], c->stream))
             return c->fail(DCP_EFAIL, "no kernel for class R=%d W=%d", sc.R, sc.W);
         if (int rc = record_launch(c, k, true, c->stream, false)) return rc;
         note_pair_launch(c, DCP_PL_QLANE_REDO, 32u, (unsigned)sc.R, (unsigned)sc.W, redo_grid[k], dcp_rowsweep_tasks_per_block(sc.W), a.pair_cap);
     }
+    a.pair_sfx = nullptr, a.sfx_buf = nullptr;
     HIP_TRY(c, hipGetLastError());
     HIP_TRY(c, hipEventRecord(c->ev_stop, c->stream));
+#ifdef DCP_TEST_HOOKS
+    c->last.sfx = qa.redo_sfx != nullptr;
+    for (int k = 0; k < kNumClasses; ++k)
+        c->last.redo_base[k] = qa.redo_base[k], c->last.redo_cap[k] = qa.redo_cap[k];
+#endif
     c->last.redo_pending = redo;
     c->last.ring_check_pending = two_stage;
     c->last.scanned = true;
@@ -3853,6 +3889,48 @@
     return DCP_OK;
 }
 
+int dcp_gpu_test_set_suffix_cap(dcp_gpu_ctx *c, unsigned long long floats)
+{
+    if (!c) return DCP_EINVAL;
+    c->sfx_cap_forced = floats;
+    return DCP_OK;
+}
+int dcp_gpu_test_last_suffix_pairs(dcp_gpu_ctx *c, unsigned *out, unsigned cap, unsigned *npairs, unsigned *without)
+{
+    if (!c || !npairs || !without) return DCP_EINVAL;
+    if (!c->last.scanned || c->last.kernel != 2 || c->last.f64) return c->fail(DCP_EINVAL, "the last scan was no float query-lane scan");
+    HIP_TRY(c, hipSetDevice(c->device));
+    HIP_TRY(c, hipStreamSynchronize(c->stream));
+    *npairs = 0, *without = 0;
+    unsigned n[DCP_MAX_CLASSES + 2] = {0};
+    if (c->d_redo_n.p) HIP_TRY(c, hipMemcpy(n, c->d_redo_n.p, sizeof n, hipMemcpyDeviceToHost));
+    if (n[DCP_MAX_CLASSES]) return c->fail(DCP_EINVAL, "a redo list of the last scan overflowed");
+    std::vector<unsigned> trip;
+    for (int k = 0; k < kNumClasses; ++k)
+    {
+        unsigned const m = std::min(n[k], c->last.redo_cap[k]);
+        if (m == 0) continue;
+        std::vector<dcp_pair> pairs(m);
+        std::vector<uint32_t> at(m, DCP_SFX_NONE);
+        HIP_TRY(c, hipMemcpy(pairs.data(), c->d_redo.p + c->last.redo_base[k], (size_t)m * sizeof(dcp_pair), hipMemcpyDeviceToHost));
+        if (c->last.sfx) HIP_TRY(c, hipMemcpy(at.data(), c->d_redo_sfx.p + c->last.redo_base[k], (size_t)m * sizeof(uint32_t), hipMemcpyDeviceToHost));
+        for (unsigned i = 0; i < m; ++i)
+        {
+            if (at[i] == DCP_SFX_NONE)
+            {
+                ++*without;
+                continue;
+            }
+            uint32_t jstar = 0;
+            HIP_TRY(c, hipMemcpy(&jstar, c->d_sfx_buf.p + at[i], sizeof jstar, hipMemcpyDeviceToHost));
+            trip.push_back(c->last.q0 + pairs[i].q), trip.push_back(c->metas[pairs[i].slot].pidx), trip.push_back(jstar);
+        }
+    }
+    *npairs = (unsigned)(trip.size() / 3u);
+    if (!out || cap < trip.size()) return trip.empty() ? DCP_OK : DCP_ENOMEM;
+    std::copy(trip.begin(), trip.end(), out);
+    return DCP_OK;
+}
 int dcp_gpu_test_set_redo_cap(dcp_gpu_ctx *c, unsigned cap)
 {
     if (!c) return DCP_EINVAL;
diff --git a/deciphon-old_amd/csrc/dcp_kernels.h b/deciphon-old_amd/csrc/dcp_kernels.h
--- a/deciphon-old_amd/csrc/dcp_kernels.h
+++ b/deciphon-old_amd/csrc/dcp_kernels.h
@@ -75,7 +75,13 @@
     float *trace_work;
     uint64_t const *trace_woff;
     float *trace_alt;
-};
+    uint32_t const *pair_sfx;
+    float const *sfx_buf;
+};
+
+#define DCP_SFX_NONE 0xffffffffu
+#define DCP_SFX_HEAD 12u
+#define DCP_SFX_WORDS(L, jstar) (DCP_SFX_HEAD + ((L) - (jstar) + 1u) + 1u)
 
 struct dcp_expand_tile
 {
@@ -165,6 +171,11 @@
     unsigned *redo_overflow;
     unsigned redo_base[DCP_MAX_CLASSES];
     unsigned redo_cap[DCP_MAX_CLASSES];
+    uint32_t *redo_sfx;
+    float *sfx_buf;
+    unsigned long long *sfx_n;
+    unsigned long long sfx_cap;
+    unsigned sfx_classes;
     float *out_null;
     float *out_alt;
     dcp_hit *hits;
diff --git a/deciphon-old_amd/csrc/dcp_kernels.hip b/deciphon-old_amd/csrc/dcp_kernels.hip
--- a/deciphon-old_amd/csrc/dcp_kernels.hip
+++ b/deciphon-old_amd/csrc/dcp_kernels.hip
@@ -244,14 +244,16 @@
 {
     template <class... A> __device__ __forceinline__ void operator()(A const &...) const {}
 };
-template <int R, int W, int PH, int PARTS = 1, class Fetch, class Sink = NoSink>
+template <int R, int W, int PH, int PARTS = 1, bool E0IN = false, class Fetch, class Sink = NoSink>
 __device__ __forceinline__ RowOut dp_row(PairState<R> &s, Trans<R> const &t,
                                          float (&em)[5][R], float (&em3)[R], float (&em4)[R], float (&em5)[R], float (&eN)[5], float (&eI)[5],
                                          LaneSpecial const &sp, float const xEB,
                                          Exchange<(W > 1 ? W : 1)> *xc,
                                          unsigned wave, unsigned lane,
-                                         unsigned &gen, unsigned const exact_e, Fetch &&fetch, Sink &&sink = Sink{})
-{
+                                         unsigned &gen, unsigned const exact_e, Fetch &&fetch, Sink &&sink = Sink{},
+                                         float const e0 = 0.0f)
+{
+    static_assert(!E0IN || (W == 1 && PARTS == 1), "a known part of E(j) is a one-wavefront pair's");
     constexpr int s1 = (PH + 4) % 5, s2 = (PH + 3) % 5, s3 = (PH + 2) % 5,
                   s4 = (PH + 1) % 5, s5 = PH;
     float const ni = neg_inf();
@@ -279,6 +281,7 @@
 #pragma unroll
         for (int r = 1; r < R; ++r)
             em = fmaxf(em, m[r]);
+        if constexpr (E0IN) em = fmaxf(em, e0);
         if constexpr (PARTS == 1) E = wave_max(em);
         else E = part_max<PARTS>(em);
     }
@@ -567,9 +570,10 @@
 {
     return W > 1 ? 64 * W : STG > 0 ? (rs_min_waves(R, W, STG == 20 && !PF) >= 4 ? 1024 : 256 * rs_min_waves(R, W, STG == 20 && !PF)) : 256;
 }
-template <int R, int W, int STG, bool PF, bool TRACE = false>
+template <int R, int W, int STG, bool PF, bool TRACE = false, bool SFX = false>
 __global__ __launch_bounds__(rs_block_threads(R, W, STG, PF), TRACE ? (W > 4 ? 1 : 2) : rs_min_waves(R, W, (STG == 20 && !PF) || (STG == 0 && W == 1 && DCP_RS_PAIR_BIG))) void viterbi_rowsweep_kernel(dcp_scan_args a)
 {
+    static_assert(!SFX || (W == 1 && STG == 0 && !PF && !TRACE), "suffix records are for the unstaged one-wavefront pair-mode kernels");
     static_assert(!PF || STG > 0, "only staged variants prefetch two rows ahead");
     static_assert(!TRACE || (STG == 0 && !PF), "the traceback's forward pass is an unstaged pair-mode kernel");
     static_assert(W == 1 || STG == 0, "only one-wavefront pairs stage rows");
@@ -594,10 +598,12 @@
     for (; task < ntasks; task += nblk * TASKS_PER_BLOCK)
     {
     unsigned slot, q0, q1;
+    unsigned sfx_at = DCP_SFX_NONE;
     if (pair_mode)
     {
         dcp_pair const pr = a.pairs[task];
         slot = pr.slot, q0 = pr.q, q1 = pr.q + 1u;
+        if constexpr (SFX) sfx_at = __builtin_amdgcn_readfirstlane(a.pair_sfx[task]);
     }
     else if constexpr (STAGED > 0)
     {
@@ -672,6 +678,18 @@
         sp.c = x == 0u ? xt[DCP_X_NB] : x == 1u ? xt[DCP_X_JB] : ni;
         float xEB = xt[DCP_X_EB];
         asm volatile("" : "+v"(xEB));
+        bool const sfx = SFX && sfx_at != DCP_SFX_NONE;
+        cfloat *rec = as_const(a.sfx_buf + (sfx ? sfx_at : 0u));
+        unsigned jb = 0u;
+        if constexpr (SFX)
+        {
+            if (sfx)
+            {
+                jb = __builtin_bit_cast(unsigned, rec[0]) - 1u;
+                if (x == 0u) sp.c = ni;
+            }
+        }
+        unsigned const Lr = L - jb;
 
         PairState<R> s;
 #pragma unroll
@@ -688,6 +706,18 @@
             for (int r = 0; r < R; ++r)
                 s.P[0][r] = B0 + t.ent[r];
             s.PX[0] = x == 0u ? 0.0f + xt[DCP_X_SN] : x == 3u ? 0.0f : ni;
+        }
+        if constexpr (SFX)
+        {
+            if (sfx)
+            {
+#pragma unroll
+                for (int r = 0; r < R; ++r)
+                    s.P[0][r] = ni;
+#pragma unroll
+                for (int i = 0; i < 5; ++i)
+                    s.PX[(i + 1) % 5] = x == 1u ? rec[2 + i] : x == 2u ? rec[7 + i] : ni;
+            }
         }
 
         float em[5][R], eN[5], eI[5];
@@ -766,29 +796,46 @@
         else
         {
         unsigned w = base_at(words, 0);
+        float e0 = ni, e0n = ni;
+        if constexpr (SFX)
+        {
+            if (sfx)
+            {
+                w = 0u;
+                for (unsigned p = jb >= 4u ? jb - 4u : 0u; p <= jb; ++p)
+                    w = (w << 2) | base_at(words, p);
+                e0 = rec[DCP_SFX_HEAD];
+            }
+        }
         load_row<R, STAGED>(em_base, ldk, lane_boff, eN_tab, eI_tab, w, em, em[2], em[3], em[4], eN, eI, stg, swd);
 
 #define DCP_ROW(PH)                                                            \
     {                                                                          \
-        w = ((w << 2) | base_at(words, j)) & 1023u;                            \
-        o = dp_row<R, W, PH>(s, t, em, em[2], em[3], em[4], eN, eI, sp, xEB, xc, wave, lane, gen, exact_e, [&]() { \
+        w = ((w << 2) | base_at(words, j + (SFX ? jb : 0u))) & 1023u;          \
+        o = dp_row<R, W, PH, 1, SFX>(s, t, em, em[2], em[3], em[4], eN, eI, sp, xEB, xc, wave, lane, gen, exact_e, [&]() { \
             load_row<R, STAGED>(em_base, ldk, lane_boff, eN_tab, eI_tab, w, em, em[2], em[3], em[4], eN, eI, stg, swd); \
-        }, sink);                                                              \
+            if constexpr (SFX) { if (sfx) e0n = rec[DCP_SFX_HEAD + j]; }       \
+        }, sink, e0);                                                          \
+        if constexpr (SFX) e0 = e0n;                                           \
         ++j;                                                                   \
     }
-        while (j + 4 <= L)
+        while (j + 4 <= Lr)
         {
             DCP_ROW(1) DCP_ROW(2) DCP_ROW(3) DCP_ROW(4) DCP_ROW(0)
         }
-        if (j <= L) DCP_ROW(1)
-        if (j <= L) DCP_ROW(2)
-        if (j <= L) DCP_ROW(3)
-        if (j <= L) DCP_ROW(4)
+        if (j <= Lr) DCP_ROW(1)
+        if (j <= Lr) DCP_ROW(2)
+        if (j <= Lr) DCP_ROW(3)
+        if (j <= Lr) DCP_ROW(4)
         }
 #undef DCP_ROW
 
         float const C = __builtin_bit_cast(float, __builtin_amdgcn_readlane(__builtin_bit_cast(int, o.X), 2));
-        float const nul = __builtin_bit_cast(float, __builtin_amdgcn_readlane(__builtin_bit_cast(int, o.X), 3));
+        float nul = __builtin_bit_cast(float, __builtin_amdgcn_readlane(__builtin_bit_cast(int, o.X), 3));
+        if constexpr (SFX)
+        {
+            if (sfx) nul = rec[1];
+        }
         float const alt = fmaxf(o.E + xt[DCP_X_ET], C + xt[DCP_X_CT]);
         if constexpr (TRACE)
         {
@@ -1642,6 +1689,14 @@
 template <int R, int W, int STG, bool PF = false>
 static void launch_rs(dcp_scan_args const *a, unsigned nblocks, unsigned threads, hipStream_t s, unsigned pad_lds = 0)
 {
+    if constexpr (W == 1 && STG == 0 && !PF)
+    {
+        if (a->pairs != nullptr && a->pair_sfx != nullptr)
+        {
+            hipLaunchKernelGGL((viterbi_rowsweep_kernel<R, W, STG, PF, false, true>), dim3(nblocks), dim3(threads), pad_lds, s, *a);
+            return;
+        }
+    }
     hipLaunchKernelGGL((viterbi_rowsweep_kernel<R, W, STG, PF>), dim3(nblocks), dim3(threads), pad_lds, s, *a);
 }
 
diff --git a/deciphon-old_amd/csrc/dcp_qlane.hip b/deciphon-old_amd/csrc/dcp_qlane.hip
--- a/deciphon-old_amd/csrc/dcp_qlane.hip
+++ b/deciphon-old_amd/csrc/dcp_qlane.hip
@@ -139,6 +139,9 @@
 {
     float B[5], Xm[5], Xd[5], Em[5];
 };
+
+template <bool SFX> using DirtyT = std::conditional_t<SFX, unsigned, bool>;
+constexpr unsigned kClean = 0xffffffffu;
 
 enum
 {
@@ -176,6 +179,7 @@
     unsigned my_flag;
     unsigned peer_flag;
     unsigned seen;
+    unsigned dummy;
 };
 constexpr unsigned kL2ImageBytes = 2u * 1364u * 16u;
 constexpr unsigned kL2TabIN = kL2ImageBytes;
@@ -340,12 +344,12 @@
 }
 
 template <int G, bool FIRST, bool LAST, int PH, int NT, int D, int IN = IO_HBM, int OUT = IO_HBM, unsigned TBASE = 0u,
-          bool IN16 = kIn16, int NV = 4 * G>
+          bool IN16 = kIn16, int NV = 4 * G, bool SFX = false>
 __device__ __forceinline__ void ql_row(QState<G> &s, TileTrans<G> const &tr, float const *tabM,
                                        float2 const *tabIN, GatherOff &go,
                                        unsigned wn, RowIn &in, Ring &ring, float *pB, float *pXm,
                                        float *pXd, float *pEm, unsigned &off, LaneXt const &xt,
-                                       bool live, bool at_end, bool &dirty, SweepOut &o,
+                                       bool live, bool at_end, DirtyT<SFX> &dirty, SweepOut &o,
                                        LdsLink const &lk, unsigned jrow, GatherMasks<TBASE> const &gm
 #if DCP_QLANE_DIAG & 4
                                        , unsigned &off2, unsigned din
@@ -369,7 +373,7 @@
     }
 
     {
-        constexpr int per_row = ((FIRST || IN != IO_HBM) ? 0 : 3) + ((LAST || OUT != IO_HBM) ? 0 : 3) +
+        constexpr int per_row = ((FIRST || IN != IO_HBM) ? 0 : 3) + (LAST ? (SFX ? 1 : 0) : OUT != IO_HBM ? 0 : 3) +
                                 ((!kRecomputeB && !FIRST) ? 1 : 0) + ((!kRecomputeB && FIRST) ? 1 : 0) + 1;
         constexpr int vm = ((D < (int)kWD ? D : (int)kWD) - 1) * per_row;
         constexpr int lgkm = kGroup1 ? 5 : 0;
@@ -525,20 +529,36 @@
         float const C = mx5(s.PC[s1] + eN[0], s.PC[s2] + eN[1], s.PC[s3] + eN[2], s.PC[s4] + eN[3],
                             s.PC[s5] + eN[4]);
         float const B1 = fmaxf(E + xt.EB, J + xt.JB);
-        dirty = dirty || (live && B1 > Bj);
-        s.PJ[PH] = fmaxf(E + xt.EJ, J + xt.JJ);
-        s.PC[PH] = fmaxf(E + xt.EC, C + xt.CC);
+        if constexpr (SFX)
+        {
+            dirty = min(dirty, (live && B1 > Bj) ? jrow : kClean);
+            bool const marked = dirty != kClean;
+            s.PJ[PH] = marked ? s.PJ[PH] : fmaxf(E + xt.EJ, J + xt.JJ);
+            s.PC[PH] = marked ? s.PC[PH] : fmaxf(E + xt.EC, C + xt.CC);
+            st_off(pEm, marked ? off : lk.dummy, E);
+        }
+        else
+        {
+            dirty = dirty || (live && B1 > Bj);
+            s.PJ[PH] = fmaxf(E + xt.EJ, J + xt.JJ);
+            s.PC[PH] = fmaxf(E + xt.EC, C + xt.CC);
+        }
         o.E = at_end ? E : o.E;
         o.C = at_end ? C : o.C;
     }
 }
 
+__device__ __forceinline__ unsigned sfx_park_off(unsigned rowbase, unsigned Lwave, unsigned NT, unsigned col, unsigned h)
+{
+    return ((rowbase + Lwave + 3u + h) * NT + col) * 4u;
+}
+
 template <int G, bool FIRST, bool LAST, int NT, int D, int IN = IO_HBM, int OUT = IO_HBM, unsigned TBASE = 0u,
-          bool IN16 = kIn16, int NV = 4 * G>
+          bool IN16 = kIn16, int NV = 4 * G, bool SFX = false>
 __device__ __forceinline__ void ql_sweep(cfloat *tt, float const *tabM, float2 const *tabIN,
                                          uint32_t const *__restrict__ wordsT, unsigned rowbase,
                                          unsigned L, unsigned Lwave, bool active, float *sc,
-                                         size_t plane, unsigned tid, LaneXt const &xt, bool &dirty,
+                                         size_t plane, unsigned tid, LaneXt const &xt, DirtyT<SFX> &dirty,
                                          SweepOut &o, LdsLink lk
 #if DCP_QLANE_DIAG & 4
                                          , unsigned tile_odd
@@ -576,6 +596,7 @@
     }
     float *pXm = sc, *pXd = sc + plane, *pEm = sc + 2 * plane, *pB = sc + (kRecomputeB ? 0 : 3) * plane;
     unsigned off = (rowbase * (unsigned)NT + tid) * 4u;
+    if constexpr (LAST && SFX) lk.dummy = ((rowbase + Lwave + 2u) * (unsigned)NT + (tid & ~63u)) * 4u;
 
     unsigned j = 1;
     static_assert(kWPlane, "the packed-word sequence planes are gone (round 4): a slot's groups are addressed by plane row");
@@ -644,7 +665,7 @@
     {                                                                                      \
                                                  \
         unsigned const pos = j + 1u;                                                       \
-        ql_row<G, FIRST, LAST, PH, NT, D, IN, OUT, TBASE, IN16, NV>(s, tr, tabM, tabIN, go,          \
+        ql_row<G, FIRST, LAST, PH, NT, D, IN, OUT, TBASE, IN16, NV, SFX>(s, tr, tabM, tabIN, go,          \
                                    (unsigned)wq[(PH + 1) % 5], in, ring, pB, pXm,                    \
                                    pXd, pEm, off, xt, active && j <= L, active && j == L,  \
                                    dirty, o, lk, rowbase + j, gm QL_DIAG4_ARGS);           \
@@ -690,6 +711,16 @@
     if (j <= Lwave) QL_ROW(3)
     if (j <= Lwave) QL_ROW(4)
 #undef QL_ROW
+    if constexpr (LAST && SFX)
+    {
+#pragma unroll
+        for (unsigned h = 0; h < 5u; ++h)
+        {
+            unsigned const po = sfx_park_off(rowbase, Lwave, (unsigned)NT, tid, h);
+            st_off(pXm, po, s.PJ[h]);
+            st_off(pXd, po, s.PC[h]);
+        }
+    }
 }
 
 template <bool IN16>
@@ -734,16 +765,20 @@
     return ((g.rowbase + g.Lwave + 8u) * NT + col) * 4u;
 }
 
-__device__ __forceinline__ void ql_publish(dcp_qlane_args const &a, dcp_ql_prof const &pm, unsigned q, float nul, float alt,
-                                           bool redo)
+__device__ __forceinline__ unsigned ql_publish(dcp_qlane_args const &a, dcp_ql_prof const &pm, unsigned q, float nul, float alt,
+                                               bool redo)
 {
     if (redo)
     {
         unsigned const cls = pm.cls;
         unsigned const i = atomicAdd(a.redo_n + cls, 1u);
-        if (i < a.redo_cap[cls]) a.redo[a.redo_base[cls] + i] = dcp_pair{q, pm.rs_slot};
-        else *a.redo_overflow = 1u;
-        return;
+        if (i < a.redo_cap[cls])
+        {
+            a.redo[a.redo_base[cls] + i] = dcp_pair{q, pm.rs_slot};
+            return a.redo_base[cls] + i;
+        }
+        *a.redo_overflow = 1u;
+        return kClean;
     }
     size_t const oi = (size_t)q * a.nprof_total + pm.pidx;
     if (a.out_null) a.out_null[oi] = nul;
@@ -752,6 +787,35 @@
     {
         unsigned const h = atomicAdd(a.nhits, 1u);
         if (h < a.hit_cap) a.hits[h] = dcp_hit{a.q_base + q, pm.pidx, nul, alt};
+    }
+    return kClean;
+}
+
+__device__ __forceinline__ void ql_cut_suffix(dcp_qlane_args const &a, float const *sc, size_t plane, unsigned NT, unsigned rowbase,
+                                              unsigned Lwave, unsigned col, unsigned lane, unsigned jstar, unsigned L, float nul,
+                                              unsigned entry)
+{
+    unsigned const n = L - jstar + 1u, len = DCP_SFX_WORDS(L, jstar);
+    unsigned long long at = 0ull;
+    if (lane == 0u) at = atomicAdd(a.sfx_n, (unsigned long long)len);
+    unsigned const lo = __builtin_amdgcn_readfirstlane((unsigned)at), hi = __builtin_amdgcn_readfirstlane((unsigned)(at >> 32));
+    at = ((unsigned long long)hi << 32) | lo;
+    if (at + len > a.sfx_cap) return;
+    float *rec = a.sfx_buf + at;
+    float const *pe = sc + 2 * plane + col;
+    if (lane < 10u)
+    {
+        unsigned const i = lane < 5u ? lane : lane - 5u;
+        rec[2u + lane] = ld_off(lane < 5u ? sc : sc + plane, sfx_park_off(rowbase, Lwave, NT, col, (jstar + i) % 5u));
+    }
+    if (lane == 10u) rec[0] = __builtin_bit_cast(float, jstar);
+    if (lane == 11u) rec[1] = nul;
+    for (unsigned i = lane; i < n; i += 64u)
+        rec[DCP_SFX_HEAD + i] = pe[(size_t)(rowbase + jstar + i - 1u) * NT];
+    if (lane == 12u)
+    {
+        rec[DCP_SFX_HEAD + n] = ninf();
+        a.redo_sfx[entry] = (unsigned)at;
     }
 }
 
@@ -834,7 +898,7 @@
     }
 }
 
-template <int G, int D, bool ROWS = false>
+template <int G, int D, bool ROWS = false, bool SFX = false>
 __global__ __launch_bounds__(512, 2) void viterbi_qlane2_kernel(dcp_qlane_args a)
 {
     constexpr int NT = (int)kRLanes;
@@ -920,9 +984,9 @@
                 t_loaded = true;
                 if (g.Lwave == 0u) continue;
                 SweepOut o{ninf(), ninf(), ninf()};
-                bool dirty = false;
+                DirtyT<SFX> dirty = SFX ? (DirtyT<SFX>)kClean : (DirtyT<SFX>)0;
 #define QL2_SWEEP_NV(F, L_, IN_, OUT_, TB_, IMG_, NV_)                                                    \
-    ql_sweep<G, F, L_, NT, D, IN_, OUT_, TB_, true, NV_>(tt, lds + ((IMG_) - (TB_)) / 4u,                  \
+    ql_sweep<G, F, L_, NT, D, IN_, OUT_, TB_, true, NV_, SFX>(tt, lds + ((IMG_) - (TB_)) / 4u,                  \
                                               reinterpret_cast<float2 const *>(lds + (kL2TabIN - (TB_)) / 4u), \
                                               wordsT, g.rowbase, g.L, g.Lwave, g.has, sc, plane, tid, g.xt, dirty, o, lk)
 #define QL2_SWEEP(F, L_, IN_, OUT_, TB_, IMG_) QL2_SWEEP_NV(F, L_, IN_, OUT_, TB_, IMG_, KT)
@@ -955,7 +1019,8 @@
                 if (last)
                 {
                     st_off(sc + plane, po, fmaxf(o.E + g.xt.ET, o.C + g.xt.CT));
-                    st_off(sc + 2 * plane, po, dirty ? 1.0f : 0.0f);
+                    if constexpr (SFX) st_off(sc + 2 * plane, po, __builtin_bit_cast(float, dirty == kClean ? 0u : (unsigned)dirty - g.rowbase));
+                    else st_off(sc + 2 * plane, po, dirty ? 1.0f : 0.0f);
                 }
             }
         }
@@ -967,12 +1032,41 @@
             cgroup *gd = (cgroup *)(unsigned long long)(a.groups + gi);
             GroupLane ge;
             ge.rowbase = gd->rowbase, ge.Lwave = gd->lmax;
-            if (ge.Lwave == 0u || (tid & 63u) >= gd->nq) continue;
-            unsigned const q = a.qorder[gd->qfirst + (tid & 63u)];
-            unsigned const po = park_off(ge, (unsigned)NT, tid);
-            float const nul = ld_off(sc, po), alt = ld_off(sc + plane, po);
-            bool const dirty = ld_off(sc + 2 * plane, po) != 0.0f;
-            ql_publish(a, pm, q, nul, alt, dirty || (kEM && pm.needs_exact_e));
+            if constexpr (!SFX)
+            {
+                if (ge.Lwave == 0u || (tid & 63u) >= gd->nq) continue;
+                unsigned const q = a.qorder[gd->qfirst + (tid & 63u)];
+                unsigned const po = park_off(ge, (unsigned)NT, tid);
+                float const nul = ld_off(sc, po), alt = ld_off(sc + plane, po);
+                bool const dirty = ld_off(sc + 2 * plane, po) != 0.0f;
+                ql_publish(a, pm, q, nul, alt, dirty || (kEM && pm.needs_exact_e));
+            }
+            else
+            {
+                if (ge.Lwave == 0u) continue;
+                unsigned const lane = tid & 63u;
+                bool const has = lane < gd->nq;
+                unsigned const q = has ? a.qorder[gd->qfirst + lane] : 0u;
+                unsigned const Lq = has ? a.seq_len[q] : 0u;
+                unsigned const po = park_off(ge, (unsigned)NT, tid);
+                float const nul = ld_off(sc, po), alt = ld_off(sc + plane, po);
+                unsigned const jstar = has ? __builtin_bit_cast(unsigned, ld_off(sc + 2 * plane, po)) : 0u;
+                bool const exact_e = kEM && pm.needs_exact_e;
+                unsigned entry = kClean;
+                if (has) entry = ql_publish(a, pm, q, nul, alt, jstar != 0u || exact_e);
+                bool const cut = a.redo_sfx != nullptr && entry != kClean && jstar != 0u && jstar <= Lq && !exact_e &&
+                                 ((a.sfx_classes >> pm.cls) & 1u) != 0u;
+                unsigned long long todo = __ballot(cut);
+                while (todo != 0ull)
+                {
+                    unsigned const l = (unsigned)__builtin_ctzll(todo);
+                    todo &= todo - 1ull;
+                    ql_cut_suffix(a, sc, plane, (unsigned)NT, ge.rowbase, ge.Lwave, (tid & ~63u) | l, lane,
+                                  (unsigned)__builtin_amdgcn_readlane((int)jstar, (int)l), (unsigned)__builtin_amdgcn_readlane((int)Lq, (int)l),
+                                  __builtin_bit_cast(float, __builtin_amdgcn_readlane(__builtin_bit_cast(int, nul), (int)l)),
+                                  (unsigned)__builtin_amdgcn_readlane((int)entry, (int)l));
+                }
+            }
         }
     }
 }
@@ -1124,6 +1218,13 @@
 
 extern "C" int dcp_launch_qlane2(dcp_qlane_args const *a, unsigned nblocks, void *stream)
 {
+    if (a->redo_sfx)
+    {
+        if (a->tiles_from_rows)
+            hipLaunchKernelGGL((viterbi_qlane2_kernel<2, DCP_QLANE_D, true, true>), dim3(nblocks), dim3(512), 0, (hipStream_t)stream, *a);
+        else hipLaunchKernelGGL((viterbi_qlane2_kernel<2, DCP_QLANE_D, false, true>), dim3(nblocks), dim3(512), 0, (hipStream_t)stream, *a);
+        return 0;
+    }
     if (a->tiles_from_rows)
         hipLaunchKernelGGL((viterbi_qlane2_kernel<2, DCP_QLANE_D, true>), dim3(nblocks), dim3(512), 0, (hipStream_t)stream, *a);
     else hipLaunchKernelGGL((viterbi_qlane2_kernel<2, DCP_QLANE_D>), dim3(nblocks), dim3(512), 0, (hipStream_t)stream, *a);
diff --git a/deciphon-old_amd/csrc/dcp_test_hooks.h b/deciphon-old_amd/csrc/dcp_test_hooks.h
--- a/deciphon-old_amd/csrc/dcp_test_hooks.h
+++ b/deciphon-old_amd/csrc/dcp_test_hooks.h
@@ -22,6 +22,8 @@
 int dcp_gpu_test_set_forward_scale_band(dcp_gpu_ctx *, unsigned bits);
 int dcp_gpu_test_set_posterior_budget(dcp_gpu_ctx *, unsigned long long bytes);
 int dcp_gpu_test_set_mea_budget(dcp_gpu_ctx *, unsigned long long bytes);
+int dcp_gpu_test_set_suffix_cap(dcp_gpu_ctx *, unsigned long long floats);
+int dcp_gpu_test_last_suffix_pairs(dcp_gpu_ctx *, unsigned *out, unsigned cap, unsigned *npairs, unsigned *without);
 }
 #endif
 
```
